# PJLab-ADG/neuralsim

Measured on NVIDIA H100. Metric: Mrays/sec fwd+bwd, higher is better.
Workload: dtype f16

## Files before the change

include/neuralsim_b200.h:

```cpp
#ifndef NEURALSIM_B200_H
#define NEURALSIM_B200_H

#include <stdint.h>

#ifdef __cplusplus
extern "C" {
#endif

#define NSB_MAX_LEVELS 32
#define NSB_MAX_DIMS 4

#define NSB_LOD_DENSE 0
#define NSB_LOD_HASH 7

typedef struct nsb_lotd_meta {
    uint32_t n_dims_to_encode;
    uint32_t n_levels;
    uint32_t n_pseudo_levels;
    uint32_t n_feat_per_pseudo_lvl;
    uint32_t n_encoded_dims;
    uint32_t n_params;
    uint32_t level_res[NSB_MAX_LEVELS][NSB_MAX_DIMS];
    uint32_t level_n_feats[NSB_MAX_LEVELS];
    uint32_t level_types[NSB_MAX_LEVELS];
    uint32_t level_sizes[NSB_MAX_LEVELS];
    uint32_t level_offsets[NSB_MAX_LEVELS + 1];
    uint32_t map_levels[NSB_MAX_LEVELS * 4];
    uint32_t map_cnt[NSB_MAX_LEVELS * 4];
} nsb_lotd_meta;

const char *nsb_last_error(void);
int nsb_version(void);
uint64_t nsb_launch_count(void);
int nsb_set_option(const char *key, int value);

int nsb_lotd_meta_create(int32_t n_dims, int32_t n_levels, const int32_t *lod_res_host,
                         const int32_t *lod_n_feats_host, const int32_t *lod_types_host,
                         uint32_t hashmap_size, nsb_lotd_meta *out_host);

int nsb_lotd_fwd(const nsb_lotd_meta *meta_host, const float *input, const void *params, int params_is_half,
                 int64_t n, int32_t max_level, void *y, float *dy_dx, void *stream);

int nsb_lotd_bwd_grid(const nsb_lotd_meta *meta_host, const void *dL_dy, int dL_dy_is_half, const float *input,
                      int64_t n, int32_t max_level, float scale, float *dL_dparam, void *stream);

int nsb_lotd_bwd_input(const void *dL_dy, int dL_dy_is_half, const float *dy_dx, int64_t n, int32_t n_feat,
                       int32_t n_dims, float scale, float *dL_dx, void *stream);

int nsb_lotd_bwd_bwd_input(const nsb_lotd_meta *meta_host, const float *dL_ddLdx, const void *dL_dy,
                           int dL_dy_is_half, const float *input, const float *dy_dx, int64_t n,
                           int32_t max_level, float scale, float *dL_ddLdy, float *dL_dparam, void *stream);

int nsb_ray_marching(int64_t n_rays, const float *rays_o, const float *rays_d, const float *t_min,
                     const float *t_max, const float *roi, const int32_t *batch_inds, int32_t rx, int32_t ry,
                     int32_t rz, const uint8_t *grid_binary, float step_size, float max_step_size,
                     float dt_gamma, uint32_t max_steps, const int32_t *packed_info, int32_t *num_steps,
                     float *t_starts, float *t_ends, int32_t *ridx, int32_t *gidx, int32_t *bidx, void *stream);
int nsb_ray_marching_listed(int64_t n_rays, const float *rays_o, const float *rays_d, const float *t_min, const float *t_max,
                            const float *roi, const int32_t *batch_inds, int32_t rx, int32_t ry, int32_t rz,
                            const uint8_t *grid_binary, float step_size, float max_step_size, float dt_gamma, uint32_t max_steps,
                            const int32_t *packed_info, int32_t *num_steps, float *t_starts, float *t_ends, int32_t *ridx,
                            int32_t *gidx, int32_t *bidx, const int64_t *ray_list, int64_t n_list, const uint32_t *grid_bits, void *stream);
int nsb_ray_marching_record(int64_t n_rays, const float *rays_o, const float *rays_d, const float *t_min, const float *t_max,
                            const float *roi, int32_t rx, int32_t ry, int32_t rz, const uint8_t *grid_binary, float step_size,
                            float max_step_size, float dt_gamma, uint32_t max_steps, int32_t *num_steps, float *rec_t,
                            const uint32_t *grid_bits, void *stream);
int nsb_march_compact(const float *rec_t, uint32_t max_steps, const int32_t *packed_info, const int64_t *ray_list, int64_t n_list,
                      float *t_starts, int32_t *ridx, void *stream);
int nsb_pack_occ_bits(const uint8_t *grid_binary, int64_t cells, uint32_t *words, void *stream);

enum { NSB_OP_ADD = 0, NSB_OP_SUB, NSB_OP_MUL, NSB_OP_DIV, NSB_OP_GT, NSB_OP_GEQ, NSB_OP_LT, NSB_OP_LEQ,
       NSB_OP_EQ, NSB_OP_NEQ };
int nsb_packed_binary(int op, const float *feats, const float *other, const int64_t *pack_infos, int64_t n_packs,
                      int32_t feat_dim, void *out, void *stream);
int nsb_packed_sum(const float *feats, const int64_t *pack_infos, int64_t n_packs, int32_t feat_dim, float *out,
                   void *stream);
int nsb_packed_cumsum(const float *feats, const int64_t *pack_infos, int64_t n_packs, int32_t feat_dim,
                      int exclusive, int reverse, float *out, void *stream);
int nsb_packed_diff(const float *feats, const int64_t *pack_infos, int64_t n_packs, int32_t feat_dim,
                    const float *appends, const float *last_fill, int backward, float *out, void *stream);
int nsb_packed_searchsorted(const float *bins, const float *vals, const int64_t *pack_infos, int64_t n_packs,
                            int32_t n_vals, int64_t *out_idx, void *stream);
int nsb_packed_invert_cdf(const float *bins, const float *cdfs, const float *u, const int64_t *pack_infos,
                          int64_t n_packs, int32_t n_samples, float *samples, int64_t *bin_idx, void *stream);
int nsb_merge_two_packs_sorted_aligned(const float *vals_a, const int64_t *pack_infos_a, const float *vals_b,
                                       const int64_t *pack_infos_b, const int64_t *pack_infos_out,
                                       int64_t n_packs, int b_sorted, int64_t *pidx_a, int64_t *pidx_b,
                                       void *stream);
int nsb_packed_alpha_to_vw_forward(const float *alphas, const int64_t *pack_infos, int64_t n_packs,
                                   float early_stop_eps, float alpha_thre, float *weights, int64_t *num_steps,
                                   uint8_t *selector, void *stream);
int nsb_packed_alpha_to_vw_backward(const float *weights, const float *grad_weights, const float *alphas,
                                    const int64_t *pack_infos, int64_t n_packs, float early_stop_eps,
                                    float alpha_thre, float *grad_alphas, void *stream);
int nsb_interleave_linstep(const float *start, const int64_t *num_steps, const int64_t *cumsum_steps,
                           const float *step_size, float step_scalar, int64_t n_packs, float *out, int64_t *nidx,
                           void *stream);
int nsb_interleave_arange(const int64_t *num_steps, const int64_t *cumsum_steps, int64_t n_packs, int64_t *out,
                          int64_t *nidx, void *stream);
int nsb_packed_sort(float *vals, const int64_t *pack_infos, int64_t n_packs, int64_t *idx, void *stream);
int nsb_mark_pack_boundaries(const int64_t *ids, int64_t n, int32_t *out, void *stream);

int nsb_sh_encode_forward(const float *inputs, float *outputs, int64_t n, int32_t degree, float *dy_dx,
                          void *stream);
int nsb_sh_encode_backward(const float *grad, const float *dy_dx, int64_t n, int32_t degree, float *grad_inputs,
                           void *stream);

typedef struct nsb_sdf_decoder {
    const void *W1;
    const void *b1;
    const void *W2;
    const void *b2;
    int32_t width;
    float beta;
} nsb_sdf_decoder;

typedef struct nsb_occ_collect {
    float *grid_pcl;
    int32_t res[3];
    float inv_s;
} nsb_occ_collect;

int nsb_fused_sdf(const nsb_lotd_meta *meta_host, const void *params_half, const nsb_sdf_decoder *dec_host,
                  const float *x, int64_t n, int32_t max_level, float *sdf, void *h_out_half, void *stream);
int nsb_fused_sdf_collect(const nsb_lotd_meta *meta_host, const void *params_half, const nsb_sdf_decoder *dec_host, const float *x,
                          const float *rays_o, const float *rays_d, const int64_t *ridx, const float *t, int64_t n,
                          const int64_t *pack_infos, const int64_t *pack_ray, const int64_t *pack_order, int64_t n_packs, int32_t mode,
                          int32_t max_level, float *sdf, const nsb_occ_collect *collect, void *stream);

int nsb_fused_sdf_rays(const nsb_lotd_meta *meta_host, const void *params_half, const nsb_sdf_decoder *dec_host,
                       const float *rays_o, const float *rays_d, const int64_t *ridx, const float *t, int64_t n,
                       int32_t max_level, float *sdf, void *stream);

int nsb_fused_sdf_packs(const nsb_lotd_meta *meta_host, const void *params_half, const nsb_sdf_decoder *dec_host, const float *rays_o,
                        const float *rays_d, const int64_t *pack_infos, const int64_t *pack_ray, int64_t n_packs, const float *t,
                        int32_t max_level, float *sdf, void *stream);

int nsb_fused_sdf_bwd(const nsb_lotd_meta *meta_host, const void *params_half, const nsb_sdf_decoder *dec_host,
                      const float *x, const float *rays_o, const float *rays_d, const int64_t *ridx, const float *t,
                      const float *d_sdf, int64_t n, int32_t max_level, float *d_grid, float *d_W1, float *d_b1,
                      float *d_W2, float *d_b2, void *stream);

int nsb_fused_sdf_bwd_indexed(const nsb_lotd_meta *meta_host, const void *params_half, const nsb_sdf_decoder *dec_host,
                              const float *x, const float *rays_o, const float *rays_d, const int64_t *ridx, const float *t,
                              const float *d_sdf, const int64_t *keep, int64_t n, int32_t max_level, float *d_grid, float *d_W1,
                              float *d_b1, float *d_W2, float *d_b2, void *stream);

int nsb_bind_device_counts(const int64_t *count0, const int64_t *count1);
int nsb_flag_nonzero(const float *v, int64_t n, int32_t *flag, void *stream);
int nsb_query_counts(int64_t *counts, int32_t phase, int32_t n_coarse, const int32_t *n_fine_host, int32_t n_stage, int64_t march_cap,
                     int64_t kept_cap, void *stream);

int nsb_neus_upsample_cdf(const float *sdf, const float *depth, const int64_t *pack_infos, int64_t n_packs, float inv_s,
                          int use_estimate_alpha, float early_stop_eps, float alpha_thre, float *cdf, void *stream);
int nsb_packed_invert_cdf_shared_u(const float *bins, const float *cdfs, const float *u, const int64_t *pack_infos, int64_t n_packs,
                                   int32_t n_samples, float *samples, void *stream);
int nsb_neus_alpha_forward(const float *sdf, const int64_t *pack_infos, int64_t n_packs, const float *inv_s_dev, float early_stop_eps,
                           float alpha_thre, float *alpha, uint8_t *selector, int32_t *num_steps, void *stream);
int nsb_neus_alpha_backward(const float *sdf, const int64_t *pack_infos, int64_t n_packs, const float *inv_s_dev, const float *d_alpha,
                            float *d_sdf, float *d_inv_s, void *stream);
int nsb_composite_forward(const float *alpha, const float *t, const float *rgb, const float *nablas, const int64_t *pack_infos,
                          int64_t n_packs, float early_stop_eps, float alpha_thre, int normalize_depth, const int64_t *ray_index,
                          float *vw, float *mask, float *depth, float *rgb_out, float *nablas_out, void *stream);
int nsb_composite_backward(const float *alpha, const float *t, const float *rgb, const float *nablas, const float *vw,
                           const int64_t *pack_infos, int64_t n_packs, float early_stop_eps, float alpha_thre, int normalize_depth,
                           const float *mask, const float *depth, const float *g_mask, const float *g_depth, const float *g_rgb,
                           const float *g_nablas, const float *g_vw, const int64_t *ray_index, float *d_alpha, float *d_rgb,
                           float *d_nablas, void *stream);

int nsb_scan_counts(const int32_t *counts, int64_t n, int32_t *first, int32_t *info2, int64_t *nz_index, int64_t *nz_pack,
                    const int64_t *src, int64_t *nz_src, int64_t *totals, const int64_t *extra_src, int64_t ticket,
                    void *workspace_zeroed, void *stream);
int64_t nsb_scan_workspace_bytes(void);
int nsb_merge_sorted_vals(const float *dep_a, const float *sdf_a, const int64_t *pack_infos_a, const float *dep_b, const float *sdf_b,
                          int64_t n_packs, int32_t n_b, float *dep_m, float *sdf_m, int64_t *pack_infos_m, void *stream);
int nsb_assemble_boundary(const float *coarse, int64_t n_rays, int32_t n_coarse, const int64_t *ridx_hit, int64_t n_hit, const float *fine,
                          int32_t n_fine, const int32_t *run_len_host, int32_t n_runs, float *d1, float *mid, int64_t *ridx_all,
                          int64_t *pack_infos, void *stream);
int nsb_compact_samples(const uint8_t *selector, const int64_t *pack_infos, const int32_t *first_out, const int32_t *kept, int64_t n_packs,
                        const int64_t *ridx_all, const float *t, const float *alpha, int64_t *pidx, int64_t *ridx_c, float *t_c,
                        float *alpha_c, void *stream);
int nsb_scatter_f32(const float *src, const int64_t *idx, int64_t n, float *dst, void *stream);
int nsb_ray_test_aabb(const float *rays_o, const float *rays_d, int64_t n, const float *center3, const float *radius3, int has_near,
                      float near_clip, int has_far, float far_clip, float *o_n, float *d_n, float *near, float *far, int32_t *flag,
                      int64_t *coherent_pairs, int64_t *row_len, void *stream);
int nsb_ray_block_order(const int64_t *pix, const int64_t *via, int64_t n_packs, int64_t n_rays, const int64_t *pairs, const int64_t *row_len,
                        int64_t *order, void *stream);
int nsb_gather_rays(const int64_t *idx, int64_t n, const float *o_n, const float *d_n, const float *near, const float *far, float *o_c,
                    float *d_c, float *near_c, float *far_c, const float *extra, float *extra_c, int32_t extra_cols, void *stream);

int nsb_occ_ema_update(const float *pts, const float *val, int64_t n, int32_t val_is_sdf, float inv_s, int32_t rx, int32_t ry, int32_t rz,
                       float *pcl_or_null, float *occ_val_grid, uint8_t *occ_grid, uint32_t *occ_bits_or_null, float ema_decay, float occ_thre,
                       float *scratch_cells, void *stream);

typedef struct nsb_color_net {
    const void *W1, *b1, *W2, *b2;
    const void *R1, *rb1, *R2, *rb2, *R3, *rb3;
    int32_t width, rad_width, rad_in, n_appear;
    float beta;
    float nablas_scale[3];
} nsb_color_net;

int64_t nsb_color_tile_bytes(int64_t n);
int nsb_fused_color_fwd(const nsb_lotd_meta *meta_host, const void *params_half, const nsb_color_net *net_host, const float *x,
                        const float *rays_o, const float *rays_d, const int64_t *ridx, const float *t, const float *view_dirs,
                        const float *h_appear, int64_t n, int32_t max_level, float *sdf, float *nablas, float *rgb, float *x_out,
                        void *act_z, void *act_x, void *act_y1, void *act_y2, const nsb_occ_collect *collect, void *stream);
int nsb_fused_color_bwd(const nsb_lotd_meta *meta_host, const void *params_half, const nsb_color_net *net_host, const float *x,
                        const float *rays_o, const float *rays_d, const int64_t *ridx, const float *t, int64_t n, int32_t max_level,
                        const void *act_z, const void *act_x, const void *act_y1, const void *act_y2, const float *rgb,
                        const float *g_sdf, const float *g_nablas, const float *g_rgb, float *dh_scratch, float *d_grid, float *d_W1,
                        float *d_b1, float *d_W2, float *d_b2, float *d_R1, float *d_rb1, float *d_R2, float *d_rb2, float *d_R3,
                        float *d_rb3, void *stream);

int nsb_upsample_rays(const nsb_lotd_meta *meta_host, const void *params_half, const nsb_sdf_decoder *dec_host, const float *rays_o,
                      const float *rays_d, const float *t_starts, const int64_t *pack_infos, const int64_t *ridx_hit, int64_t n_hit,
                      int32_t max_level, int32_t n_stage, const int32_t *n_fine_host, const float *inv_s_stage_host,
                      const float *const *u_stage_host, int32_t use_estimate_alpha, float early_stop_eps, float alpha_thre, float *fine_all,
                      int32_t *overflow, float *scratch, int32_t long_cap, const nsb_occ_collect *collect, void *stream);
int64_t nsb_upsample_rays_scratch_floats(int64_t n_hit_capacity, int32_t long_cap);
int nsb_upsample_persistent(const nsb_lotd_meta *meta_host, const void *params_half, const nsb_sdf_decoder *dec_host, const float *rays_o,
                            const float *rays_d, const float *t_starts, const int64_t *pack_infos, const int64_t *ridx_hit, int64_t n_hit,
                            int32_t max_level, int32_t n_stage, const int32_t *n_fine, const float *inv_s_stage, const float *const *u_stage,
                            int32_t use_estimate_alpha, float early_stop_eps, float alpha_thre, float *fine_all, int32_t *overflow, void *stream);

int nsb_mc_lattice_points(const float *lin0, const float *lin1, const float *lin2, int32_t n1, int32_t n2, int64_t start, int64_t n, float *x,
                          void *stream);
int nsb_mc_count(const float *sdf_win, int32_t w0, int32_t n_win, int32_t n0, int32_t n1, int32_t n2, int32_t p0, int32_t p1, double level,
                 uint8_t *flags, int32_t *vcount, uint8_t *cases, int32_t *tcount, void *stream);
int nsb_mc_vertices(const float *sdf_win, int32_t w0, int32_t n_win, int32_t n0, int32_t n1, int32_t n2, int32_t p0, int32_t p1, double level,
                    const double *bmin3_host, const double *spacing3_host, const uint8_t *flags, const int32_t *vfirst, float *verts, float *normals,
                    void *stream);
int nsb_mc_triangles(int32_t n0, int32_t n1, int32_t n2, int32_t p0, int32_t p1, const uint8_t *cases, const int32_t *tcount, const int32_t *tfirst,
                     const uint8_t *flags, const int32_t *vfirst, int64_t vbase, const uint8_t *carry_flags, const int32_t *carry_first,
                     int64_t carry_base, int32_t *faces, void *stream);

#ifdef __cplusplus
}
#endif
#endif
```

neuralsim_b200/csrc/neus_fused.cu:

```cuda
#include "neus_device.cuh"

namespace nsb {

constexpr int kNB = 256;
__device__ __forceinline__ int64_t gwarp() { return ((int64_t)blockIdx.x * blockDim.x + threadIdx.x) >> 5; }
__device__ __forceinline__ int64_t nwarps() { return ((int64_t)gridDim.x * blockDim.x) >> 5; }
inline unsigned pack_grid(int64_t n_packs) { return wave_grid(n_packs * 32, kNB, 8); }

__global__ void __launch_bounds__(kNB)
k_upsample_cdf(const float *__restrict__ sdf, const float *__restrict__ dep, const int64_t *__restrict__ pi, int64_t n_packs, float inv_s,
               int use_estimate, float eps, float thre, float *__restrict__ cdf, const int64_t *__restrict__ n_dev) {
    const int lane = threadIdx.x & 31;
    n_packs = eff_n(n_packs, n_dev);
    for (int64_t p = gwarp(); p < n_packs; p += nwarps()) {
        const int64_t b = pi[2 * p], n = pi[2 * p + 1];
        float T = 1.f, carry = 0.f, last_excl = 0.f;
        bool stopped = false;
        int cnt = 0;
        for (int64_t k0 = 0; k0 < n; k0 += 32) {
            const int64_t k = k0 + lane;
            float a = 0.f;
            if (k < n) a = use_estimate ? upsample_alpha_at(sdf, dep, b, n, k, inv_s) : neus_alpha_at(sdf, b, n, k, inv_s);
            float w;
            bool sel;
            replay_chunk(a, (int)min((int64_t)32, n - k0), lane, eps, thre, T, stopped, cnt, w, sel);
            const float inc = warp_scan_incl(w, lane) + carry;
            const float excl = inc - w;
            if (k < n) cdf[b + k] = excl;
            if (k == n - 1) last_excl = excl;
            carry = __shfl_sync(0xffffffffu, inc, 31);
        }
        last_excl = __shfl_sync(0xffffffffu, last_excl, (int)((n - 1) & 31));
        const float norm = fmaxf(last_excl, 1e-5f);
        __syncwarp();
        for (int64_t k = lane; k < n; k += 32) cdf[b + k] = __fdiv_rn(cdf[b + k], norm);
    }
}

__global__ void __launch_bounds__(256)
k_invert_cdf_shared_u(const float *__restrict__ bins, const float *__restrict__ cdfs, const float *__restrict__ u, const int64_t *__restrict__ pi,
                      int64_t n_packs, int n_s, float *__restrict__ samples, const int64_t *__restrict__ n_dev) {
    n_packs = eff_n(n_packs, n_dev);
    const int64_t total = n_packs * n_s, stride = (int64_t)gridDim.x * blockDim.x;
    for (int64_t t = (int64_t)blockIdx.x * blockDim.x + threadIdx.x; t < total; t += stride) {
        const int64_t p = t / n_s;
        const int64_t b = pi[2 * p];
        const uint32_t n = (uint32_t)pi[2 * p + 1];
        if (n == 0) { samples[t] = __int_as_float(0x7fc00000); continue; }
        const float *bb = bins + b, *cc = cdfs + b;
        const float uu = u[t - p * n_s];
        uint32_t first = 0, count = n;
        while (count > 0) {
            const uint32_t step = count >> 1, it = first + step;
            if (cc[it] < uu) { first = it + 1; count -= step + 1; } else count = step;
        }
        const uint32_t pos = min(first, n - 1);
        float r;
        if (pos == 0) r = bb[0];
        else {
            const float c0 = cc[pos - 1], pmf = __fsub_rn(cc[pos], c0);
            r = pmf < 1.0e-5f ? bb[pos - 1] : __fmaf_rn(__fdiv_rn(__fsub_rn(uu, c0), pmf), __fsub_rn(bb[pos], bb[pos - 1]), bb[pos - 1]);
        }
        samples[t] = r;
    }
}

__global__ void __launch_bounds__(kNB)
k_neus_alpha_fwd(const float *__restrict__ sdf, const int64_t *__restrict__ pi, int64_t n_packs, const float *__restrict__ inv_s_p, float eps,
                 float thre, float *__restrict__ alpha, uint8_t *__restrict__ selector, int32_t *__restrict__ num_steps,
                 const int64_t *__restrict__ n_dev) {
    const int lane = threadIdx.x & 31;
    const float inv_s = inv_s_p[0];
    if (n_dev) {
        const int64_t live = eff_n(n_packs, n_dev);
        for (int64_t p = live + (int64_t)blockIdx.x * blockDim.x + threadIdx.x; p < n_packs; p += (int64_t)gridDim.x * blockDim.x) num_steps[p] = 0;
        n_packs = live;
    }
    for (int64_t p = gwarp(); p < n_packs; p += nwarps()) {
        const int64_t b = pi[2 * p], n = pi[2 * p + 1];
        float T = 1.f;
        bool stopped = false;
        int cnt = 0;
        for (int64_t k0 = 0; k0 < n; k0 += 32) {
            const int64_t k = k0 + lane;
            const float a = (k < n) ? neus_alpha_at(sdf, b, n, k, inv_s) : 0.f;
            float w;
            bool sel;
            replay_chunk(a, (int)min((int64_t)32, n - k0), lane, eps, thre, T, stopped, cnt, w, sel);
            if (k < n) { alpha[b + k] = a; selector[b + k] = sel ? 1 : 0; }
        }
        if (lane == 0) num_steps[p] = cnt;
    }
}

__global__ void __launch_bounds__(kNB)
k_neus_alpha_bwd(const float *__restrict__ sdf, const int64_t *__restrict__ pi, int64_t n_packs, const float *__restrict__ inv_s_p,
                 const float *__restrict__ d_alpha, float *__restrict__ d_sdf, float *__restrict__ d_inv_s, const int64_t *__restrict__ n_dev) {
    const int lane = threadIdx.x & 31;
    const float inv_s = inv_s_p[0];
    n_packs = eff_n(n_packs, n_dev);
    float acc_invs = 0.f;
    for (int64_t p = gwarp(); p < n_packs; p += nwarps()) {
        const int64_t b = pi[2 * p], n = pi[2 * p + 1];
        for (int64_t k = lane; k < n; k += 32) {
            const float g_own = (k < n - 1) ? d_alpha[b + k] : 0.f, g_prev = (k > 0) ? d_alpha[b + k - 1] : 0.f;
            if (g_own == 0.f && g_prev == 0.f) { d_sdf[b + k] = 0.f; continue; }
            const float s = sdf[b + k];
            const float c = sigmoidf_(s * inv_s);
            float gc = 0.f;
            if (k < n - 1) {
                const float c1 = sigmoidf_(sdf[b + k + 1] * inv_s);
                const float den = c + 1e-5f;
                if ((c - c1) / den >= 0.f) gc += g_own * (c1 + 1e-5f) / (den * den);
            }
            if (k > 0) {
                const float cp = sigmoidf_(sdf[b + k - 1] * inv_s);
                const float den = cp + 1e-5f;
                if ((cp - c) / den >= 0.f) gc -= g_prev / den;
            }
            const float dc = c * (1.f - c);
            d_sdf[b + k] = gc * dc * inv_s;
            acc_invs += gc * dc * s;
        }
    }
    acc_invs = warp_sum(acc_invs);
    if (lane == 0 && acc_invs != 0.f) atomicAdd(d_inv_s, acc_invs);
}

__global__ void __launch_bounds__(kNB)
k_composite_fwd(const float *__restrict__ alpha, const float *__restrict__ t, const float *__restrict__ rgb, const float *__restrict__ nab,
                const int64_t *__restrict__ pi, int64_t n_packs, float eps, float thre, int normalize_depth, const int64_t *__restrict__ ray_index,
                float *__restrict__ vw, float *__restrict__ mask, float *__restrict__ depth, float *__restrict__ rgb_out, float *__restrict__ nab_out,
                const int64_t *__restrict__ n_dev) {
    const int lane = threadIdx.x & 31;
    n_packs = eff_n(n_packs, n_dev);
    for (int64_t p = gwarp(); p < n_packs; p += nwarps()) {
        const int64_t b = pi[2 * p], n = pi[2 * p + 1];
        float T = 1.f;
        bool stopped = false;
        int cnt = 0;
        float sm = 0.f, sd = 0.f, sr[3] = {0.f, 0.f, 0.f}, sn[3] = {0.f, 0.f, 0.f};
        for (int64_t k0 = 0; k0 < n; k0 += 32) {
            const int64_t k = k0 + lane;
            const float a = (k < n) ? alpha[b + k] : 0.f;
            float w;
            bool sel;
            replay_chunk(a, (int)min((int64_t)32, n - k0), lane, eps, thre, T, stopped, cnt, w, sel);
            if (k < n) {
                vw[b + k] = w;
                sm += w;
                sd = fmaf(w, t[b + k], sd);
                if (rgb) { sr[0] = fmaf(w, rgb[(b + k) * 3], sr[0]); sr[1] = fmaf(w, rgb[(b + k) * 3 + 1], sr[1]); sr[2] = fmaf(w, rgb[(b + k) * 3 + 2], sr[2]); }
                if (nab) { sn[0] = fmaf(w, nab[(b + k) * 3], sn[0]); sn[1] = fmaf(w, nab[(b + k) * 3 + 1], sn[1]); sn[2] = fmaf(w, nab[(b + k) * 3 + 2], sn[2]); }
            }
        }
        sm = warp_sum(sm); sd = warp_sum(sd);
#pragma unroll
        for (int c = 0; c < 3; ++c) { sr[c] = warp_sum(sr[c]); sn[c] = warp_sum(sn[c]); }
        if (lane == 0) {
            const int64_t o = ray_index ? ray_index[p] : p;
            mask[o] = sm;
            depth[o] = normalize_depth ? sd / (sm + 1e-10f) : sd;
            if (rgb) { rgb_out[o * 3] = sr[0]; rgb_out[o * 3 + 1] = sr[1]; rgb_out[o * 3 + 2] = sr[2]; }
            if (nab) { nab_out[o * 3] = sn[0]; nab_out[o * 3 + 1] = sn[1]; nab_out[o * 3 + 2] = sn[2]; }
        }
    }
}

__global__ void __launch_bounds__(kNB)
k_composite_bwd(const float *__restrict__ alpha, const float *__restrict__ t, const float *__restrict__ rgb, const float *__restrict__ nab,
                const float *__restrict__ vw, const int64_t *__restrict__ pi, int64_t n_packs, float eps, float thre, int normalize_depth,
                const float *__restrict__ mask, const float *__restrict__ depth, const float *__restrict__ g_mask, const float *__restrict__ g_depth,
                const float *__restrict__ g_rgb, const float *__restrict__ g_nab, const float *__restrict__ g_vw_ext,
                const int64_t *__restrict__ ray_index, float *__restrict__ d_alpha, float *__restrict__ d_rgb, float *__restrict__ d_nab,
                const int64_t *__restrict__ n_dev) {
    const int lane = threadIdx.x & 31;
    n_packs = eff_n(n_packs, n_dev);
    for (int64_t p = gwarp(); p < n_packs; p += nwarps()) {
        const int64_t b = pi[2 * p], n = pi[2 * p + 1];
        const int64_t o = ray_index ? ray_index[p] : p;
        const float gm = g_mask ? g_mask[o] : 0.f, gd = g_depth ? g_depth[o] : 0.f;
        const float M = mask[o], Dp = depth[o];
        const float inv = normalize_depth ? 1.f / (M + 1e-10f) : 1.f;
        float gr[3] = {0.f, 0.f, 0.f}, gn[3] = {0.f, 0.f, 0.f};
        if (g_rgb) { gr[0] = g_rgb[o * 3]; gr[1] = g_rgb[o * 3 + 1]; gr[2] = g_rgb[o * 3 + 2]; }
        if (g_nab) { gn[0] = g_nab[o * 3]; gn[1] = g_nab[o * 3 + 1]; gn[2] = g_nab[o * 3 + 2]; }
        float accum = 0.f;
        for (int64_t k = lane; k < n; k += 32) {
            const float w = vw[b + k];
            float gw = gm + gd * (normalize_depth ? (t[b + k] - Dp) * inv : t[b + k]);
            if (g_vw_ext) gw += g_vw_ext[b + k];
            if (rgb) {
                gw += gr[0] * rgb[(b + k) * 3] + gr[1] * rgb[(b + k) * 3 + 1] + gr[2] * rgb[(b + k) * 3 + 2];
                d_rgb[(b + k) * 3] = w * gr[0]; d_rgb[(b + k) * 3 + 1] = w * gr[1]; d_rgb[(b + k) * 3 + 2] = w * gr[2];
            }
            if (nab) {
                gw += gn[0] * nab[(b + k) * 3] + gn[1] * nab[(b + k) * 3 + 1] + gn[2] * nab[(b + k) * 3 + 2];
                d_nab[(b + k) * 3] = w * gn[0]; d_nab[(b + k) * 3 + 1] = w * gn[1]; d_nab[(b + k) * 3 + 2] = w * gn[2];
            }
            d_alpha[b + k] = gw;
            accum += gw * w;
        }
        accum = warp_sum(accum);
        __syncwarp();
        float T = 1.f;
        bool stopped = false;
        for (int64_t k0 = 0; k0 < n; k0 += 32) {
            const int64_t k = k0 + lane;
            const float a = (k < n) ? alpha[b + k] : 0.f;
            const float gw = (k < n) ? d_alpha[b + k] : 0.f;
            const float gww = (k < n) ? gw * vw[b + k] : 0.f;
            float my_g = 0.f;
            if (!stopped) {
                const int lim = (int)min((int64_t)32, n - k0);
                for (int q = 0; q < lim; ++q) {
                    const float aq = __shfl_sync(0xffffffffu, a, q);
                    const float gq = __shfl_sync(0xffffffffu, gww, q);
                    if (T < eps) { stopped = true; break; }
                    if (aq < thre) continue;
                    if (q == lane) my_g = __fdiv_rn(gw * T - accum, fmaxf(1.f - aq, 1e-10f));
                    accum -= gq;
                    T *= (1.f - aq);
                }
            }
            if (k < n) d_alpha[b + k] = my_g;
        }
    }
}

}

using namespace nsb;
#define STREAM ((cudaStream_t)stream)

extern "C" int nsb_neus_upsample_cdf(const float *sdf, const float *depth, const int64_t *pack_infos, int64_t n_packs, float inv_s,
                                     int use_estimate_alpha, float early_stop_eps, float alpha_thre, float *cdf, void *stream) {
    const DevCounts dn = take_counts();
    if (n_packs == 0) return 0;
    NSB_REQUIRE(sdf && depth && pack_infos && cdf, "nsb_neus_upsample_cdf: NULL argument");
    k_upsample_cdf<<<pack_grid(n_packs), kNB, 0, STREAM>>>(sdf, depth, pack_infos, n_packs, inv_s, use_estimate_alpha, early_stop_eps, alpha_thre, cdf, dn.a);
    return check_launch("nsb_neus_upsample_cdf");
}

extern "C" int nsb_packed_invert_cdf_shared_u(const float *bins, const float *cdfs, const float *u, const int64_t *pack_infos, int64_t n_packs,
                                              int32_t n_samples, float *samples, void *stream) {
    const DevCounts dn = take_counts();
    if (n_packs == 0 || n_samples == 0) return 0;
    NSB_REQUIRE(bins && cdfs && u && pack_infos && samples, "nsb_packed_invert_cdf_shared_u: NULL argument");
    k_invert_cdf_shared_u<<<wave_grid(n_packs * n_samples, 256, 8), 256, 0, STREAM>>>(bins, cdfs, u, pack_infos, n_packs, n_samples, samples, dn.a);
    return check_launch("nsb_packed_invert_cdf_shared_u");
}

extern "C" int nsb_neus_alpha_forward(const float *sdf, const int64_t *pack_infos, int64_t n_packs, const float *inv_s_dev, float early_stop_eps,
                                      float alpha_thre, float *alpha, uint8_t *selector, int32_t *num_steps, void *stream) {
    const DevCounts dn = take_counts();
    if (n_packs == 0) return 0;
    NSB_REQUIRE(sdf && pack_infos && inv_s_dev && alpha && selector && num_steps, "nsb_neus_alpha_forward: NULL argument");
    k_neus_alpha_fwd<<<pack_grid(n_packs), kNB, 0, STREAM>>>(sdf, pack_infos, n_packs, inv_s_dev, early_stop_eps, alpha_thre, alpha, selector, num_steps, dn.a);
    return check_launch("nsb_neus_alpha_forward");
}

extern "C" int nsb_neus_alpha_backward(const float *sdf, const int64_t *pack_infos, int64_t n_packs, const float *inv_s_dev, const float *d_alpha,
                                       float *d_sdf, float *d_inv_s, void *stream) {
    const DevCounts dn = take_counts();
    if (n_packs == 0) return 0;
    NSB_REQUIRE(sdf && pack_infos && inv_s_dev && d_alpha && d_sdf && d_inv_s, "nsb_neus_alpha_backward: NULL argument");
    k_neus_alpha_bwd<<<pack_grid(n_packs), kNB, 0, STREAM>>>(sdf, pack_infos, n_packs, inv_s_dev, d_alpha, d_sdf, d_inv_s, dn.a);
    return check_launch("nsb_neus_alpha_backward");
}

extern "C" int nsb_composite_forward(const float *alpha, const float *t, const float *rgb, const float *nablas, const int64_t *pack_infos,
                                     int64_t n_packs, float early_stop_eps, float alpha_thre, int normalize_depth, const int64_t *ray_index,
                                     float *vw, float *mask, float *depth, float *rgb_out, float *nablas_out, void *stream) {
    const DevCounts dn = take_counts();
    if (n_packs == 0) return 0;
    NSB_REQUIRE(alpha && t && pack_infos && vw && mask && depth, "nsb_composite_forward: NULL argument");
    NSB_REQUIRE((!rgb || rgb_out) && (!nablas || nablas_out), "nsb_composite_forward: missing output buffer");
    k_composite_fwd<<<pack_grid(n_packs), kNB, 0, STREAM>>>(alpha, t, rgb, nablas, pack_infos, n_packs, early_stop_eps, alpha_thre, normalize_depth,
                                                            ray_index, vw, mask, depth, rgb_out, nablas_out, dn.a);
    return check_launch("nsb_composite_forward");
}

extern "C" int nsb_composite_backward(const float *alpha, const float *t, const float *rgb, const float *nablas, const float *vw,
                                      const int64_t *pack_infos, int64_t n_packs, float early_stop_eps, float alpha_thre, int normalize_depth,
                                      const float *mask, const float *depth, const float *g_mask, const float *g_depth, const float *g_rgb,
                                      const float *g_nablas, const float *g_vw, const int64_t *ray_index, float *d_alpha, float *d_rgb,
                                      float *d_nablas, void *stream) {
    const DevCounts dn = take_counts();
    if (n_packs == 0) return 0;
    NSB_REQUIRE(alpha && t && vw && pack_infos && mask && depth && d_alpha, "nsb_composite_backward: NULL argument");
    NSB_REQUIRE((!rgb || d_rgb) && (!nablas || d_nablas), "nsb_composite_backward: missing output buffer");
    k_composite_bwd<<<pack_grid(n_packs), kNB, 0, STREAM>>>(alpha, t, rgb, nablas, vw, pack_infos, n_packs, early_stop_eps, alpha_thre, normalize_depth,
                                                            mask, depth, g_mask, g_depth, g_rgb, g_nablas, g_vw, ray_index, d_alpha, d_rgb, d_nablas, dn.a);
    return check_launch("nsb_composite_backward");
}
```

neuralsim_b200/csrc/neus_glue.cu:

```cuda
#include "nsb_common.cuh"

namespace nsb {

__device__ __forceinline__ int64_t gwarp_() { return ((int64_t)blockIdx.x * blockDim.x + threadIdx.x) >> 5; }
__device__ __forceinline__ int64_t nwarps_() { return ((int64_t)gridDim.x * blockDim.x) >> 5; }

constexpr int kScanT = 1024, kScanI = 8, kScanMaxBlocks = 128;
struct ScanWs {
    long long sum[kScanMaxBlocks];
    int nz[kScanMaxBlocks];
    int flag[kScanMaxBlocks];
    int ticket;
};

__device__ __forceinline__ void block_scan_pair(int64_t &ps, int32_t &pz, int lane, int warp, int64_t *s_sum, int32_t *s_nz) {
#pragma unroll
    for (int o = 1; o < 32; o <<= 1) {
        const int64_t a = __shfl_up_sync(0xffffffffu, ps, o);
        const int32_t b = __shfl_up_sync(0xffffffffu, pz, o);
        if (lane >= o) { ps += a; pz += b; }
    }
    __syncthreads();
    if (lane == 31) { s_sum[warp] = ps; s_nz[warp] = pz; }
    __syncthreads();
    if (warp == 0) {
        int64_t a = s_sum[lane];
        int32_t b = s_nz[lane];
#pragma unroll
        for (int o = 1; o < 32; o <<= 1) {
            const int64_t a2 = __shfl_up_sync(0xffffffffu, a, o);
            const int32_t b2 = __shfl_up_sync(0xffffffffu, b, o);
            if (lane >= o) { a += a2; b += b2; }
        }
        s_sum[lane] = a;
        s_nz[lane] = b;
    }
    __syncthreads();
}

__global__ void __launch_bounds__(kScanT)
k_scan_counts(const int32_t *__restrict__ counts, int64_t n, int64_t seg, ScanWs *__restrict__ ws, int32_t *__restrict__ first,
              int32_t *__restrict__ info2, int64_t *__restrict__ nz_index, int64_t *__restrict__ nz_pack, const int64_t *__restrict__ src,
              int64_t *__restrict__ nz_src, int64_t *totals, const int64_t *__restrict__ extra_src, int64_t ticket) {
    __shared__ int64_t s_sum[32];
    __shared__ int32_t s_nz[32];
    __shared__ int64_t s_carry_sum;
    __shared__ int32_t s_carry_nz;
    __shared__ int s_b;
    if (threadIdx.x == 0) s_b = atomicAdd(&ws->ticket, 1);
    __syncthreads();
    const int tid = threadIdx.x, lane = tid & 31, warp = tid >> 5, b = s_b;
    const int64_t lo = (int64_t)b * seg, hi = min(n, lo + seg);
    int64_t ps = 0;
    int32_t pz = 0;
    for (int64_t i = lo + tid; i < hi; i += kScanT) { const int32_t c = counts[i]; ps += c; pz += c > 0 ? 1 : 0; }
    block_scan_pair(ps, pz, lane, warp, s_sum, s_nz);
    const int64_t my_sum = s_sum[31];
    const int32_t my_nz = s_nz[31];
    if (tid == 0) {
        ws->sum[b] = my_sum;
        ws->nz[b] = my_nz;
        __threadfence();
        atomicExch(&ws->flag[b], 1);
    }
    ps = 0;
    pz = 0;
    if (tid < b) {
        while (atomicAdd(&ws->flag[tid], 0) == 0) {}
        __threadfence();
        ps = *((volatile long long *)&ws->sum[tid]);
        pz = *((volatile int *)&ws->nz[tid]);
    }
    block_scan_pair(ps, pz, lane, warp, s_sum, s_nz);
    if (tid == 0) { s_carry_sum = s_sum[31]; s_carry_nz = s_nz[31]; }
    __syncthreads();
    int64_t carry_sum = s_carry_sum;
    int32_t carry_nz = s_carry_nz;
    if (b == gridDim.x - 1 && tid == 0) {
        volatile int64_t *tv = totals;
        tv[0] = carry_sum + my_sum;
        tv[1] = carry_nz + my_nz;
        if (extra_src) tv[2] = extra_src[0];
        if (ticket) {
            __threadfence_system();
            tv[3] = ticket;
        }
    }
    for (int64_t base = lo; base < hi; base += (int64_t)kScanT * kScanI) {
        const int64_t i0 = base + (int64_t)tid * kScanI;
        int32_t c[kScanI];
        ps = 0;
        pz = 0;
#pragma unroll
        for (int k = 0; k < kScanI; ++k) {
            c[k] = (i0 + k < hi) ? counts[i0 + k] : 0;
            ps += c[k];
            pz += c[k] > 0 ? 1 : 0;
        }
        const int64_t tsum = ps;
        const int32_t tnz = pz;
        block_scan_pair(ps, pz, lane, warp, s_sum, s_nz);
        int64_t excl = carry_sum + (warp ? s_sum[warp - 1] : 0) + ps - tsum;
        int32_t rank = carry_nz + (warp ? s_nz[warp - 1] : 0) + pz - tnz;
#pragma unroll
        for (int k = 0; k < kScanI; ++k) {
            const int64_t i = i0 + k;
            if (i < hi) {
                if (first) first[i] = (int32_t)excl;
                if (info2) { info2[2 * i] = (int32_t)excl; info2[2 * i + 1] = c[k]; }
                if (c[k] > 0) {
                    if (nz_index) nz_index[rank] = i;
                    if (nz_pack) { nz_pack[2 * rank] = excl; nz_pack[2 * rank + 1] = c[k]; }
                    if (nz_src) nz_src[rank] = src[i];
                    ++rank;
                }
            }
            excl += c[k];
        }
        carry_sum += s_sum[31];
        carry_nz += s_nz[31];
    }
}

constexpr int kMergeWarps = 8;
__global__ void __launch_bounds__(kMergeWarps * 32)
k_merge_vals(const float *__restrict__ dep_a, const float *__restrict__ sdf_a, const int64_t *__restrict__ pi_a, const float *__restrict__ dep_b,
             const float *__restrict__ sdf_b, int64_t n_packs, int nb, float *__restrict__ dep_m, float *__restrict__ sdf_m,
             int64_t *__restrict__ pi_m, const int64_t *__restrict__ n_dev) {
    extern __shared__ float s_b[];
    n_packs = eff_n(n_packs, n_dev);
    const int lane = threadIdx.x & 31, w = threadIdx.x >> 5;
    float *bb = s_b + w * nb;
    for (int64_t p = gwarp_(); p < n_packs; p += nwarps_()) {
        const int64_t a0 = pi_a[2 * p], na = pi_a[2 * p + 1];
        const int64_t m0 = a0 + p * nb;
        __syncwarp();
        for (int j = lane; j < nb; j += 32) bb[j] = dep_b[p * nb + j];
        __syncwarp();
        if (lane == 0) { pi_m[2 * p] = m0; pi_m[2 * p + 1] = na + nb; }
        for (int64_t i = lane; i < na; i += 32) {
            const float v = dep_a[a0 + i];
            int lo = 0, cnt = nb;
            while (cnt > 0) {
                const int step = cnt >> 1;
                if (bb[lo + step] <= v) { lo += step + 1; cnt -= step + 1; } else cnt = step;
            }
            dep_m[m0 + i + lo] = v;
            if (sdf_m) sdf_m[m0 + i + lo] = sdf_a[a0 + i];
        }
        for (int j = lane; j < nb; j += 32) {
            const float v = bb[j];
            int64_t lo = 0, cnt = na;
            while (cnt > 0) {
                const int64_t step = cnt >> 1;
                if (dep_a[a0 + lo + step] < v) { lo += step + 1; cnt -= step + 1; } else cnt = step;
            }
            dep_m[m0 + j + lo] = v;
            if (sdf_m) sdf_m[m0 + j + lo] = sdf_b[p * nb + j];
        }
    }
}

constexpr int kAsmWarps = 8, kAsmMaxRuns = 8, kAsmChunk = 8;
struct AsmRuns { int n, len[kAsmMaxRuns]; };

__device__ __forceinline__ int count_less(const float *a, int n, float v, bool or_equal) {
    int lo = 0, cnt = n;
    while (cnt > 0) {
        const int step = cnt >> 1;
        const float u = a[lo + step];
        if (or_equal ? (u <= v) : (u < v)) { lo += step + 1; cnt -= step + 1; } else cnt = step;
    }
    return lo;
}

__global__ void __launch_bounds__(kAsmWarps * 32)
k_assemble_boundary(const float *__restrict__ coarse, int64_t n_rays, int nc, const int64_t *__restrict__ ridx_hit, int64_t n_hit,
                    const float *__restrict__ fine, int nf, const AsmRuns runs, float *__restrict__ d1, float *__restrict__ mid,
                    int64_t *__restrict__ ridx_all, int64_t *__restrict__ pack_infos, const int64_t *__restrict__ n_rays_dev,
                    const int64_t *__restrict__ n_hit_dev) {
    extern __shared__ float s_v[];
    static_assert(kAsmChunk >= 1 && kAsmChunk <= 32, "one candidate per lane");
    n_rays = eff_n(n_rays, n_rays_dev);
    n_hit = eff_n(n_hit, n_hit_dev);
    const int lane = threadIdx.x & 31, w = threadIdx.x >> 5, cap = nc + nf;
    float *raw = s_v + (size_t)w * 2 * cap, *srt = raw + cap;
    const int64_t n_chunks = (n_rays + kAsmChunk - 1) / kAsmChunk;
    for (int64_t c = gwarp_(); c < n_chunks; c += nwarps_()) {
        const int64_t r0 = c * kAsmChunk;
        int64_t lo0 = 0, cnt = n_hit;
        while (cnt > 0) {
            const int64_t step = cnt >> 1;
            if (ridx_hit[lo0 + step] < r0) { lo0 += step + 1; cnt -= step + 1; } else cnt = step;
        }
        long long cand = -1;
        if (lane < kAsmChunk && lo0 + lane < n_hit) cand = ridx_hit[lo0 + lane];
        int used = 0;
        for (int j = 0; j < kAsmChunk; ++j) {
            const int64_t r = r0 + j;
            if (r >= n_rays) break;
            const bool hit = __shfl_sync(0xffffffffu, cand, used) == r;
            const int64_t lo = lo0 + used;
            const int n = nc + (hit ? nf : 0);
            const int64_t first = (int64_t)nc * r + (int64_t)nf * lo;
            if (lane == 0) { pack_infos[2 * r] = first; pack_infos[2 * r + 1] = n; }
            if (!hit) {
                for (int k = lane; k < nc; k += 32) {
                    const float v = coarse[r * nc + k];
                    const float diff = (k < nc - 1) ? __fsub_rn(coarse[r * nc + k + 1], v) : 0.f;
                    d1[first + k] = v;
                    mid[first + k] = __fadd_rn(v, __fmul_rn(diff, 0.5f));
                    ridx_all[first + k] = r;
                }
                continue;
            }
            ++used;
            __syncwarp();
            for (int k = lane; k < nc; k += 32) raw[k] = coarse[r * nc + k];
            for (int k = lane; k < nf; k += 32) raw[nc + k] = fine[lo * nf + k];
            __syncwarp();
            for (int e = lane; e < n; e += 32) {
                const float v = raw[e];
                int rank = 0, start = 0;
                for (int q = -1; q < runs.n; ++q) {
                    const int len = q < 0 ? nc : runs.len[q];
                    if (e >= start && e < start + len) rank += e - start;
                    else rank += count_less(raw + start, len, v, start < e);
                    start += len;
                }
                srt[rank] = v;
            }
            __syncwarp();
            for (int k = lane; k < n; k += 32) {
                const float v = srt[k];
                const float diff = (k < n - 1) ? __fsub_rn(srt[k + 1], v) : 0.f;
                d1[first + k] = v;
                mid[first + k] = __fadd_rn(v, __fmul_rn(diff, 0.5f));
                ridx_all[first + k] = r;
            }
        }
    }
}

__global__ void __launch_bounds__(256)
k_compact_samples(const uint8_t *__restrict__ selector, const int64_t *__restrict__ pi, const int32_t *__restrict__ first_out,
                  const int32_t *__restrict__ kept, int64_t n_packs, const int64_t *__restrict__ ridx_all, const float *__restrict__ t,
                  const float *__restrict__ alpha, int64_t *__restrict__ pidx, int64_t *__restrict__ ridx_c, float *__restrict__ t_c,
                  float *__restrict__ alpha_c, const int64_t *__restrict__ n_dev) {
    const int lane = threadIdx.x & 31;
    n_packs = eff_n(n_packs, n_dev);
    for (int64_t p = gwarp_(); p < n_packs; p += nwarps_()) {
        const int32_t kp = kept[p];
        if (kp == 0) continue;
        const int64_t b = pi[2 * p], n = pi[2 * p + 1];
        int64_t out = first_out[p];
        int32_t done = 0;
        for (int64_t k0 = 0; k0 < n && done < kp; k0 += 32) {
            const int64_t k = k0 + lane;
            const bool sel = k < n && selector[b + k] != 0;
            const uint32_t m = __ballot_sync(0xffffffffu, sel);
            if (sel) {
                const int64_t o = out + __popc(m & ((1u << lane) - 1u));
                pidx[o] = b + k;
                ridx_c[o] = ridx_all[b + k];
                t_c[o] = t[b + k];
                alpha_c[o] = alpha[b + k];
            }
            const int c = __popc(m);
            out += c;
            done += c;
        }
    }
}

__global__ void __launch_bounds__(256)
k_scatter_f32(const float *__restrict__ src, const int64_t *__restrict__ idx, int64_t n, float *__restrict__ dst, const int64_t *__restrict__ n_dev) {
    n = eff_n(n, n_dev);
    const int64_t stride = (int64_t)gridDim.x * blockDim.x;
    for (int64_t j = (int64_t)blockIdx.x * blockDim.x + threadIdx.x; j < n; j += stride) dst[idx[j]] = src[j];
}


__device__ __forceinline__ float min_nan(float a, float b) { return (a != a || b != b) ? __int_as_float(0x7fc00000) : fminf(a, b); }
__device__ __forceinline__ float max_nan(float a, float b) { return (a != a || b != b) ? __int_as_float(0x7fc00000) : fmaxf(a, b); }

struct RayTestArgs {
    float c[3], r[3];
    float near_clip, far_clip;
    int has_near, has_far;
};

__global__ void __launch_bounds__(256)
k_ray_test_aabb(const float *__restrict__ rays_o, const float *__restrict__ rays_d, int64_t n, const RayTestArgs a, float *__restrict__ o_n,
                float *__restrict__ d_n, float *__restrict__ near, float *__restrict__ far, int32_t *__restrict__ flag,
                unsigned long long *__restrict__ coherent_pairs, unsigned long long *__restrict__ row_len) {
    const int64_t stride = (int64_t)gridDim.x * blockDim.x;
    unsigned int close = 0;
    for (int64_t i = (int64_t)blockIdx.x * blockDim.x + threadIdx.x; i < n; i += stride) {
        if (row_len && i >= 2) {
            float rev = 0.f;
#pragma unroll
            for (int d = 0; d < 3; ++d) rev += (rays_d[i * 3 + d] - rays_d[(i - 1) * 3 + d]) * (rays_d[3 + d] - rays_d[d]);
            if (rev < 0.f) atomicMin(row_len, (unsigned long long)i);
        }
        if (coherent_pairs && i > 0) {
            float dd = 0.f, od = 0.f;
#pragma unroll
            for (int d = 0; d < 3; ++d) {
                dd = fmaxf(dd, fabsf(rays_d[i * 3 + d] - rays_d[(i - 1) * 3 + d]));
                od = fmaxf(od, fabsf(rays_o[i * 3 + d] - rays_o[(i - 1) * 3 + d]) / a.r[d]);
            }
            const float len = fmaxf(fmaxf(fabsf(rays_d[i * 3]), fabsf(rays_d[i * 3 + 1])), fabsf(rays_d[i * 3 + 2]));
            close += (dd <= 0.03f * len && od <= 0.03f) ? 1u : 0u;
        }
        float tn = 0.f, tf = 0.f;
#pragma unroll
        for (int d = 0; d < 3; ++d) {
            const float o = __fdiv_rn(__fsub_rn(rays_o[i * 3 + d], a.c[d]), a.r[d]);
            const float v = __fdiv_rn(rays_d[i * 3 + d], a.r[d]);
            o_n[i * 3 + d] = o;
            d_n[i * 3 + d] = v;
            const float ta = __fdiv_rn(__fsub_rn(-1.f, o), v), tb = __fdiv_rn(__fsub_rn(1.f, o), v);
            const float lo = min_nan(ta, tb), hi = max_nan(ta, tb);
            tn = d == 0 ? lo : max_nan(tn, lo);
            tf = d == 0 ? hi : min_nan(tf, hi);
        }
        if (a.has_near && tn == tn) tn = fmaxf(tn, a.near_clip);
        if (a.has_far && tf == tf) tf = fminf(tf, a.far_clip);
        bool m = (tf > tn) && (tf > (a.has_near ? a.near_clip : 0.f));
        if (a.has_far) m = m && (tn < a.far_clip);
        near[i] = tn;
        far[i] = tf;
        flag[i] = m ? 1 : 0;
    }
    if (coherent_pairs) {
        close = __reduce_add_sync(0xffffffffu, close);
        if ((threadIdx.x & 31) == 0 && close) atomicAdd(coherent_pairs, (unsigned long long)close);
    }
}

constexpr int kOrdT = 256, kOrdMaxBx = 4096;
constexpr int kBlkW = 8, kBlkH = 4;

__device__ __forceinline__ int64_t pixel_of(const int64_t *__restrict__ pix, const int64_t *__restrict__ via, int64_t p) {
    return pix[via ? via[p] : p];
}

__device__ int64_t lower_bound_pixel(const int64_t *__restrict__ pix, const int64_t *__restrict__ via, int64_t n, int64_t key) {
    int64_t lo = 0, hi = n;
    while (lo < hi) {
        const int64_t mid = (lo + hi) >> 1;
        if (pixel_of(pix, via, mid) < key) lo = mid + 1; else hi = mid;
    }
    return lo;
}

__global__ void __launch_bounds__(kOrdT)
k_ray_block_order(const int64_t *__restrict__ pix, const int64_t *__restrict__ via, int64_t n, int64_t n_rays, const int64_t *__restrict__ pairs,
                  const int64_t *__restrict__ row_len, int64_t *__restrict__ order, const int64_t *__restrict__ n_dev) {
    __shared__ uint32_t mask[kOrdMaxBx];
    __shared__ int32_t offs[kOrdMaxBx];
    __shared__ int32_t wsum[kOrdT / 32];
    n = eff_n(n, n_dev);
    const int64_t W = *row_len;
    const bool coherent = n_rays > 64 && 4 * *pairs >= 3 * (n_rays - 1);
    const int64_t nbx = (W + kBlkW - 1) / kBlkW;
    const int tid = threadIdx.x, lane = tid & 31, warp = tid >> 5;
    if (n == 0) return;
    if (!coherent || W < 2 || nbx > kOrdMaxBx) {
        for (int64_t j = (int64_t)blockIdx.x * kOrdT + tid; j < n; j += (int64_t)gridDim.x * kOrdT) order[j] = j;
        return;
    }
    const int64_t rows = kBlkH * W, n_brows = pixel_of(pix, via, n - 1) / rows + 1;
    constexpr int kPer = kOrdMaxBx / kOrdT;
    for (int64_t by = blockIdx.x; by < n_brows; by += gridDim.x) {
        const int64_t lo = lower_bound_pixel(pix, via, n, by * rows), hi = lower_bound_pixel(pix, via, n, (by + 1) * rows);
        for (int64_t b = tid; b < nbx; b += kOrdT) mask[b] = 0u;
        __syncthreads();
        for (int64_t p = lo + tid; p < hi; p += kOrdT) {
            const int64_t q = pixel_of(pix, via, p) - by * rows, py = q / W, px = q - py * W;
            atomicOr(&mask[px / kBlkW], 1u << (py * kBlkW + px % kBlkW));
        }
        __syncthreads();
        int loc = 0;
#pragma unroll
        for (int k = 0; k < kPer; ++k) {
            const int b = tid * kPer + k;
            if (b < nbx) loc += __popc(mask[b]);
        }
        int incl = loc;
#pragma unroll
        for (int o = 1; o < 32; o <<= 1) {
            const int v = __shfl_up_sync(0xffffffffu, incl, o);
            if (lane >= o) incl += v;
        }
        if (lane == 31) wsum[warp] = incl;
        __syncthreads();
        int run = incl - loc;
        for (int w = 0; w < warp; ++w) run += wsum[w];
#pragma unroll
        for (int k = 0; k < kPer; ++k) {
            const int b = tid * kPer + k;
            if (b < nbx) { offs[b] = run; run += __popc(mask[b]); }
        }
        __syncthreads();
        for (int64_t p = lo + tid; p < hi; p += kOrdT) {
            const int64_t q = pixel_of(pix, via, p) - by * rows, py = q / W, px = q - py * W;
            const uint32_t bit = (uint32_t)(py * kBlkW + px % kBlkW);
            order[lo + offs[px / kBlkW] + __popc(mask[px / kBlkW] & ((1u << bit) - 1u))] = p;
        }
        __syncthreads();
    }
}

__global__ void __launch_bounds__(256)
k_gather_rays(const int64_t *__restrict__ idx, int64_t n, const float *__restrict__ o_n, const float *__restrict__ d_n, const float *__restrict__ near,
              const float *__restrict__ far, float *__restrict__ o_c, float *__restrict__ d_c, float *__restrict__ near_c, float *__restrict__ far_c,
              const float *__restrict__ extra, float *__restrict__ extra_c, int extra_cols, const int64_t *__restrict__ n_dev) {
    n = eff_n(n, n_dev);
    const int64_t stride = (int64_t)gridDim.x * blockDim.x;
    for (int64_t j = (int64_t)blockIdx.x * blockDim.x + threadIdx.x; j < n; j += stride) {
        const int64_t i = idx[j];
#pragma unroll
        for (int d = 0; d < 3; ++d) { o_c[j * 3 + d] = o_n[i * 3 + d]; d_c[j * 3 + d] = d_n[i * 3 + d]; }
        near_c[j] = near[i];
        far_c[j] = far[i];
        for (int c = 0; c < extra_cols; ++c) extra_c[j * extra_cols + c] = extra[i * extra_cols + c];
    }
}

__global__ void __launch_bounds__(256)
k_flag_nonzero(const float *__restrict__ v, int64_t n, int32_t *__restrict__ flag, const int64_t *__restrict__ n_dev) {
    const int64_t ne = eff_n(n, n_dev), stride = (int64_t)gridDim.x * blockDim.x;
    for (int64_t i = (int64_t)blockIdx.x * blockDim.x + threadIdx.x; i < n; i += stride) flag[i] = (i < ne && v[i] != 0.f) ? 1 : 0;
}

__global__ void k_query_counts(int64_t *__restrict__ c, int phase, int nc, int n_stage, int nf0, int nf1, int nf2, int nf3, int64_t march_cap,
                               int64_t kept_cap) {
    if (threadIdx.x != 0 || blockIdx.x != 0) return;
    if (phase == 0) {
        const int nf[4] = {nf0, nf1, nf2, nf3};
        int64_t M = c[3], nh = c[4];
        int64_t worst = M, tot = 0;
        for (int q = 0; q + 1 < n_stage; ++q) worst += nh * nf[q];
        if (worst > march_cap) { c[20] |= 1; M = 0; nh = 0; }
        c[12] = M;
        c[13] = nh;
        int64_t merged = M;
        for (int q = 0; q < 4; ++q) {
            c[14 + q] = q < n_stage ? nh * nf[q] : 0;
            if (q < n_stage) tot += nf[q];
            if (q + 1 < n_stage) merged += nh * nf[q];
            c[22 + q] = merged;
        }
        c[18] = c[0] * nc + nh * tot;
    } else {
        int64_t K = c[6], pu = c[7];
        const bool fits = K <= kept_cap;
        if (!fits) { c[20] |= 2; K = 0; pu = 0; }
        c[19] = K;
        c[21] = pu;
        c[26] = fits ? c[0] : 0;
    }
}

}

using namespace nsb;
#define STREAM ((cudaStream_t)stream)

extern "C" int nsb_flag_nonzero(const float *v, int64_t n, int32_t *flag, void *stream) {
    const DevCounts dn = take_counts();
    if (n == 0) return 0;
    NSB_REQUIRE(v && flag, "nsb_flag_nonzero: NULL argument");
    k_flag_nonzero<<<wave_grid(n, 256, 8), 256, 0, STREAM>>>(v, n, flag, dn.a);
    return check_launch("nsb_flag_nonzero");
}

extern "C" int nsb_query_counts(int64_t *counts, int32_t phase, int32_t n_coarse, const int32_t *n_fine_host, int32_t n_stage, int64_t march_cap,
                                int64_t kept_cap, void *stream) {
    NSB_REQUIRE(counts, "nsb_query_counts: counts is NULL");
    NSB_REQUIRE(n_stage >= 0 && n_stage <= 4 && (n_stage == 0 || n_fine_host), "nsb_query_counts: at most 4 up-sampling stages");
    int nf[4] = {0, 0, 0, 0};
    for (int q = 0; q < n_stage; ++q) nf[q] = n_fine_host[q];
    k_query_counts<<<1, 32, 0, STREAM>>>(counts, phase, n_coarse, n_stage, nf[0], nf[1], nf[2], nf[3], march_cap, kept_cap);
    return check_launch("nsb_query_counts");
}

extern "C" int64_t nsb_scan_workspace_bytes(void) { return (int64_t)sizeof(ScanWs); }

extern "C" int nsb_scan_counts(const int32_t *counts, int64_t n, int32_t *first, int32_t *info2, int64_t *nz_index, int64_t *nz_pack,
                               const int64_t *src, int64_t *nz_src, int64_t *totals, const int64_t *extra_src, int64_t ticket,
                               void *workspace_zeroed, void *stream) {
    NSB_REQUIRE(totals && workspace_zeroed, "nsb_scan_counts: totals / workspace is NULL");
    NSB_REQUIRE(n == 0 || counts, "nsb_scan_counts: counts is NULL");
    NSB_REQUIRE(!nz_src || src, "nsb_scan_counts: nz_src needs src");
    int64_t nb = (n + (int64_t)kScanT * kScanI - 1) / ((int64_t)kScanT * kScanI);
    const int64_t cap = sm_count() < kScanMaxBlocks ? sm_count() : kScanMaxBlocks;
    if (nb > cap) nb = cap;
    if (nb < 1) nb = 1;
    int64_t seg = (n + nb - 1) / nb;
    seg = (seg + kScanI - 1) / kScanI * kScanI;
    k_scan_counts<<<(unsigned)nb, kScanT, 0, STREAM>>>(counts, n, seg, (ScanWs *)workspace_zeroed, first, info2, nz_index, nz_pack, src, nz_src, totals, extra_src, ticket);
    return check_launch("nsb_scan_counts");
}

extern "C" int nsb_merge_sorted_vals(const float *dep_a, const float *sdf_a, const int64_t *pack_infos_a, const float *dep_b, const float *sdf_b,
                                     int64_t n_packs, int32_t n_b, float *dep_m, float *sdf_m, int64_t *pack_infos_m, void *stream) {
    const DevCounts dn = take_counts();
    if (n_packs == 0) return 0;
    NSB_REQUIRE(dep_a && pack_infos_a && dep_b && dep_m && pack_infos_m, "nsb_merge_sorted_vals: NULL argument");
    NSB_REQUIRE((sdf_m == nullptr) || (sdf_a && sdf_b), "nsb_merge_sorted_vals: sdf_m needs sdf_a and sdf_b");
    NSB_REQUIRE(n_b > 0 && n_b <= 1024, "nsb_merge_sorted_vals: n_b must be in [1, 1024]");
    const size_t smem = (size_t)kMergeWarps * n_b * sizeof(float);
    k_merge_vals<<<wave_grid(n_packs * 32, kMergeWarps * 32, 8), kMergeWarps * 32, smem, STREAM>>>(dep_a, sdf_a, pack_infos_a, dep_b, sdf_b, n_packs, n_b,
                                                                                                 dep_m, sdf_m, pack_infos_m, dn.a);
    return check_launch("nsb_merge_sorted_vals");
}

extern "C" int nsb_assemble_boundary(const float *coarse, int64_t n_rays, int32_t n_coarse, const int64_t *ridx_hit, int64_t n_hit, const float *fine,
                                     int32_t n_fine, const int32_t *run_len, int32_t n_runs, float *d1, float *mid, int64_t *ridx_all,
                                     int64_t *pack_infos, void *stream) {
    const DevCounts dn = take_counts();
    if (n_rays == 0) return 0;
    NSB_REQUIRE(coarse && d1 && mid && ridx_all && pack_infos, "nsb_assemble_boundary: NULL argument");
    NSB_REQUIRE(n_hit == 0 || (ridx_hit && fine), "nsb_assemble_boundary: hit rays need ridx_hit and fine");
    NSB_REQUIRE(n_coarse > 0 && n_fine >= 0 && n_coarse + n_fine <= 1024, "nsb_assemble_boundary: n_coarse + n_fine must be <= 1024");
    const size_t smem = (size_t)kAsmWarps * 2 * (n_coarse + n_fine) * sizeof(float);
    NSB_REQUIRE(smem <= 96 * 1024, "nsb_assemble_boundary: too many samples per ray for shared memory");
    AsmRuns runs{};
    NSB_REQUIRE(n_runs >= 0 && n_runs <= kAsmMaxRuns && (n_runs == 0 || run_len), "nsb_assemble_boundary: at most %d sorted runs", kAsmMaxRuns);
    int tot = 0;
    for (int q = 0; q < n_runs; ++q) { runs.len[q] = run_len[q]; tot += run_len[q]; }
    runs.n = n_runs;
    NSB_REQUIRE(tot == n_fine, "nsb_assemble_boundary: run lengths must add up to n_fine");
    const unsigned grid = wave_grid(n_rays * 32, kAsmWarps * 32, 8);
    opt_in_smem(k_assemble_boundary, 96 * 1024);
    k_assemble_boundary<<<grid, kAsmWarps * 32, smem, STREAM>>>(coarse, n_rays, n_coarse, ridx_hit, n_hit, fine, n_fine, runs, d1, mid, ridx_all, pack_infos,
                                                               dn.a, dn.b);
    return check_launch("nsb_assemble_boundary");
}

extern "C" int nsb_compact_samples(const uint8_t *selector, const int64_t *pack_infos, const int32_t *first_out, const int32_t *kept, int64_t n_packs,
                                   const int64_t *ridx_all, const float *t, const float *alpha, int64_t *pidx, int64_t *ridx_c, float *t_c,
                                   float *alpha_c, void *stream) {
    const DevCounts dn = take_counts();
    if (n_packs == 0) return 0;
    NSB_REQUIRE(selector && pack_infos && first_out && kept && ridx_all && t && alpha && pidx && ridx_c && t_c && alpha_c,
                "nsb_compact_samples: NULL argument");
    k_compact_samples<<<wave_grid(n_packs * 32, 256, 8), 256, 0, STREAM>>>(selector, pack_infos, first_out, kept, n_packs, ridx_all, t, alpha, pidx, ridx_c,
                                                                          t_c, alpha_c, dn.a);
    return check_launch("nsb_compact_samples");
}

extern "C" int nsb_scatter_f32(const float *src, const int64_t *idx, int64_t n, float *dst, void *stream) {
    const DevCounts dn = take_counts();
    if (n == 0) return 0;
    NSB_REQUIRE(src && idx && dst, "nsb_scatter_f32: NULL argument");
    k_scatter_f32<<<wave_grid(n, 256, 8), 256, 0, STREAM>>>(src, idx, n, dst, dn.a);
    return check_launch("nsb_scatter_f32");
}

extern "C" int nsb_ray_test_aabb(const float *rays_o, const float *rays_d, int64_t n, const float *center3, const float *radius3, int has_near,
                                 float near_clip, int has_far, float far_clip, float *o_n, float *d_n, float *near, float *far, int32_t *flag,
                                 int64_t *coherent_pairs, int64_t *row_len, void *stream) {
    if (n == 0) return 0;
    NSB_REQUIRE(rays_o && rays_d && center3 && radius3 && o_n && d_n && near && far && flag, "nsb_ray_test_aabb: NULL argument");
    RayTestArgs a{{center3[0], center3[1], center3[2]}, {radius3[0], radius3[1], radius3[2]}, near_clip, far_clip, has_near, has_far};
    if (row_len && cudaMemsetAsync(row_len, 0xff, sizeof(int64_t), STREAM) != cudaSuccess) return check_launch("nsb_ray_test_aabb (row length)");
    k_ray_test_aabb<<<wave_grid(n, 256, 8), 256, 0, STREAM>>>(rays_o, rays_d, n, a, o_n, d_n, near, far, flag, (unsigned long long *)coherent_pairs,
                                                           (unsigned long long *)row_len);
    return check_launch("nsb_ray_test_aabb");
}

extern "C" int nsb_ray_block_order(const int64_t *pix, const int64_t *via, int64_t n_packs, int64_t n_rays, const int64_t *pairs, const int64_t *row_len,
                                   int64_t *order, void *stream) {
    const DevCounts dn = take_counts();
    if (n_packs == 0) return 0;
    NSB_REQUIRE(pix && pairs && row_len && order, "nsb_ray_block_order: NULL argument");
    k_ray_block_order<<<wave_grid(n_packs, 4 * 32 * 8, 1), kOrdT, 0, STREAM>>>(pix, via, n_packs, n_rays, pairs, row_len, order, dn.a);
    return check_launch("nsb_ray_block_order");
}

extern "C" int nsb_gather_rays(const int64_t *idx, int64_t n, const float *o_n, const float *d_n, const float *near, const float *far, float *o_c,
                               float *d_c, float *near_c, float *far_c, const float *extra, float *extra_c, int32_t extra_cols, void *stream) {
    const DevCounts dn = take_counts();
    if (n == 0) return 0;
    NSB_REQUIRE(idx && o_n && d_n && near && far && o_c && d_c && near_c && far_c, "nsb_gather_rays: NULL argument");
    NSB_REQUIRE(extra_cols == 0 || (extra && extra_c), "nsb_gather_rays: extra payload needs both pointers");
    k_gather_rays<<<wave_grid(n, 256, 8), 256, 0, STREAM>>>(idx, n, o_n, d_n, near, far, o_c, d_c, near_c, far_c, extra, extra_c, extra_cols, dn.a);
    return check_launch("nsb_gather_rays");
}
```

neuralsim_b200/graphics/neus_fused.py:

```python
from __future__ import annotations

import ctypes

import torch

from .. import _lib as L

__all__ = ["upsample_cdf", "sample_cdf_uniform", "neus_alpha_compress", "neus_alpha_compact", "composite", "scan_counts", "merge_sorted_vals",
           "assemble_boundary", "march_lean", "upsample_rays", "block_order"]

_U_CACHE = {}


def _f32c(t):
    return t.detach().contiguous().float()


@torch.no_grad()
def upsample_cdf(sdf, depth, pack_infos, inv_s: float, use_estimate_alpha=False, early_stop_eps=1e-4, alpha_thre=0.0):
    sdf, depth = _f32c(sdf), _f32c(depth)
    cdf = torch.empty_like(sdf)
    L.check(L.lib().nsb_neus_upsample_cdf(L.ptr(sdf, "f32"), L.ptr(depth, "f32"), L.ptr(pack_infos, "i64"), L.c_i64(pack_infos.shape[0]),
                                          L.c_f32(inv_s), ctypes.c_int(1 if use_estimate_alpha else 0), L.c_f32(early_stop_eps),
                                          L.c_f32(alpha_thre), L.ptr(cdf), L.stream_ptr()), "neus_upsample_cdf")
    return cdf


@torch.no_grad()
def sample_cdf_uniform(bins, cdfs, pack_infos, num_to_sample: int):
    key = (num_to_sample, bins.device)
    u = _U_CACHE.get(key)
    if u is None:
        u = _U_CACHE[key] = torch.linspace(0., 1., num_to_sample + 2, device=bins.device, dtype=torch.float32)[1:-1].contiguous()
    P = pack_infos.shape[0]
    out = torch.empty(P, num_to_sample, device=bins.device, dtype=torch.float32)
    L.check(L.lib().nsb_packed_invert_cdf_shared_u(L.ptr(bins, "f32"), L.ptr(cdfs, "f32"), L.ptr(u, "f32"), L.ptr(pack_infos, "i64"),
                                                   L.c_i64(P), L.c_i32(num_to_sample), L.ptr(out), L.stream_ptr()),
            "packed_invert_cdf_shared_u")
    return out


class _NeusAlpha(torch.autograd.Function):
    @staticmethod
    def forward(ctx, sdf, inv_s, pack_infos, early_stop_eps, alpha_thre):
        sdf_c, inv_c = _f32c(sdf), _f32c(inv_s).reshape(1)
        P = pack_infos.shape[0]
        alpha = torch.empty_like(sdf_c)
        sel = torch.empty(sdf_c.shape[0], dtype=torch.bool, device=sdf_c.device)
        steps = torch.empty(P, dtype=torch.int32, device=sdf_c.device)
        L.check(L.lib().nsb_neus_alpha_forward(L.ptr(sdf_c, "f32"), L.ptr(pack_infos, "i64"), L.c_i64(P), L.ptr(inv_c, "f32"),
                                               L.c_f32(early_stop_eps), L.c_f32(alpha_thre), L.ptr(alpha), L.ptr(sel), L.ptr(steps),
                                               L.stream_ptr()), "neus_alpha_forward")
        ctx.save_for_backward(sdf_c, inv_c, pack_infos)
        ctx.inv_shape = inv_s.shape
        ctx.mark_non_differentiable(sel, steps)
        return alpha, sel, steps

    @staticmethod
    def backward(ctx, g_alpha, _gs, _gn):
        sdf_c, inv_c, pack_infos = ctx.saved_tensors
        g = g_alpha.contiguous().float()
        d_sdf = torch.empty_like(sdf_c)
        d_inv = torch.zeros(1, device=sdf_c.device, dtype=torch.float32)
        L.check(L.lib().nsb_neus_alpha_backward(L.ptr(sdf_c, "f32"), L.ptr(pack_infos, "i64"), L.c_i64(pack_infos.shape[0]),
                                                L.ptr(inv_c, "f32"), L.ptr(g, "f32"), L.ptr(d_sdf), L.ptr(d_inv), L.stream_ptr()),
                "neus_alpha_backward")
        return (d_sdf if ctx.needs_input_grad[0] else None, d_inv.reshape(ctx.inv_shape) if ctx.needs_input_grad[1] else None,
                None, None, None)


def neus_alpha_compress(sdf, inv_s, pack_infos, early_stop_eps=1e-4, alpha_thre=0.0):
    if not isinstance(inv_s, torch.Tensor):
        inv_s = torch.tensor(float(inv_s), device=sdf.device)
    alpha, sel, steps = _NeusAlpha.apply(sdf, inv_s, pack_infos, early_stop_eps, alpha_thre)
    pidx = sel.nonzero()[..., 0]
    nidx = (steps > 0).nonzero()[..., 0]
    kept = steps[nidx].long()
    cs = kept.cumsum(0)
    return alpha, nidx, torch.stack([cs - kept, kept], 1), pidx


class _GatherUnique(torch.autograd.Function):

    @staticmethod
    def forward(ctx, src, pidx, gathered):
        ctx.save_for_backward(pidx)
        ctx.n = src.shape[0]
        return gathered

    @staticmethod
    def backward(ctx, g):
        pidx, = ctx.saved_tensors
        g = g.contiguous().float()
        d = torch.zeros(ctx.n, dtype=torch.float32, device=g.device)
        L.check(L.lib().nsb_scatter_f32(L.ptr(g, "f32"), L.ptr(pidx, "i64"), L.c_i64(pidx.shape[0]), L.ptr(d), L.stream_ptr()), "scatter_f32")
        return d, None, None


_SCAN_WS = []
_HOST_SLOTS = {}


def _host_slot():
    dev = torch.cuda.current_device()
    st = _HOST_SLOTS.get(dev)
    if st is None:
        t = torch.zeros(4, dtype=torch.int64).pin_memory()
        st = _HOST_SLOTS[dev] = [t, t.numpy(), 0]
    return st


def _scan_ws_bytes():
    if not _SCAN_WS:
        L.lib().nsb_scan_workspace_bytes.restype = ctypes.c_int64
        _SCAN_WS.append(int(L.lib().nsb_scan_workspace_bytes()))
    return _SCAN_WS[0]


@torch.no_grad()
def scan_counts(counts, *, want_first=False, want_info2=False, want_index=False, want_pack=False, src=None, extra=None):
    n, dev = counts.shape[0], counts.device
    first = torch.empty(n, dtype=torch.int32, device=dev) if want_first else None
    info2 = torch.empty(n, 2, dtype=torch.int32, device=dev) if want_info2 else None
    index = torch.empty(n, dtype=torch.int64, device=dev) if want_index else None
    pack = torch.empty(n, 2, dtype=torch.int64, device=dev) if want_pack else None
    nz_src = torch.empty(n, dtype=torch.int64, device=dev) if src is not None else None
    slot = _host_slot()
    slot[2] += 1
    ticket = slot[2]
    ws = torch.zeros(_scan_ws_bytes(), dtype=torch.uint8, device=dev)
    L.check(L.lib().nsb_scan_counts(L.ptr(counts, "i32"), L.c_i64(n), L.ptr(first, allow_none=True), L.ptr(info2, allow_none=True),
                                    L.ptr(index, allow_none=True), L.ptr(pack, allow_none=True), L.ptr(src, "i64", allow_none=True),
                                    L.ptr(nz_src, allow_none=True), ctypes.c_void_p(slot[0].data_ptr()), L.ptr(extra, "i64", allow_none=True),
                                    L.c_i64(ticket), L.ptr(ws), L.stream_ptr()), "scan_counts")
    host = slot[1]
    spins = 0
    while host[3] != ticket:
        spins += 1
        if spins > 2_000_000 and spins % 1_000_000 == 0:
            torch.cuda.current_stream().synchronize()
            if host[3] != ticket:
                raise RuntimeError("scan_counts: the kernel finished without publishing its totals")
    total, nnz = int(host[0]), int(host[1])
    out = dict(total=total, n_nonzero=nnz, first=first, info2=info2, extra=[int(host[2])])
    out["index"] = index[:nnz] if index is not None else None
    out["pack"] = pack[:nnz] if pack is not None else None
    out["src"] = nz_src[:nnz] if nz_src is not None else None
    return out


@torch.no_grad()
def block_order(pix, via, rays_row):
    n = pix.shape[0] if via is None else via.shape[0]
    order = torch.empty(n, dtype=torch.int64, device=pix.device)
    n_rays, pr = rays_row
    L.check(L.lib().nsb_ray_block_order(L.ptr(pix, "i64"), L.ptr(via, "i64", allow_none=True), L.c_i64(n), L.c_i64(n_rays), L.ptr(pr, "i64"),
                                        L.ptr(pr[1:], "i64"), L.ptr(order), L.stream_ptr()), "ray_block_order")
    return order


@torch.no_grad()
def merge_sorted_vals(dep_a, sdf_a, pack_infos_a, dep_b, sdf_b):
    P, nb = dep_b.shape
    n = dep_a.shape[0] + P * nb
    dep_m = torch.empty(n, dtype=torch.float32, device=dep_a.device)
    sdf_m = torch.empty_like(dep_m) if sdf_a is not None else None
    pim = torch.empty_like(pack_infos_a)
    L.check(L.lib().nsb_merge_sorted_vals(L.ptr(dep_a, "f32"), L.ptr(sdf_a, "f32", allow_none=True), L.ptr(pack_infos_a, "i64"), L.ptr(dep_b, "f32"),
                                          L.ptr(sdf_b, "f32", allow_none=True), L.c_i64(P), L.c_i32(nb), L.ptr(dep_m), L.ptr(sdf_m, allow_none=True),
                                          L.ptr(pim), L.stream_ptr()), "merge_sorted_vals")
    return dep_m, sdf_m, pim


@torch.no_grad()
def assemble_boundary(coarse, ridx_hit, fine, run_len=None):
    R, nc = coarse.shape
    n_hit, nf = (fine.shape if fine is not None else (0, 0))
    S, dev = R * nc + n_hit * nf, coarse.device
    d1, mid = torch.empty(S, dtype=torch.float32, device=dev), torch.empty(S, dtype=torch.float32, device=dev)
    ridx_all = torch.empty(S, dtype=torch.int64, device=dev)
    pi = torch.empty(R, 2, dtype=torch.int64, device=dev)
    run_len = [nf] if run_len is None else list(run_len)
    rl = (ctypes.c_int32 * len(run_len))(*run_len)
    L.check(L.lib().nsb_assemble_boundary(L.ptr(coarse, "f32"), L.c_i64(R), L.c_i32(nc), L.ptr(ridx_hit, "i64", allow_none=True), L.c_i64(n_hit),
                                          L.ptr(fine, "f32", allow_none=True), L.c_i32(nf), rl, L.c_i32(len(run_len)), L.ptr(d1), L.ptr(mid),
                                          L.ptr(ridx_all), L.ptr(pi), L.stream_ptr()), "assemble_boundary")
    return d1, mid, ridx_all, pi


def neus_alpha_compact(sdf, inv_s, pack_infos, ridx_all, t_mid, rays_inds, early_stop_eps=1e-4, alpha_thre=0.0):
    if not isinstance(inv_s, torch.Tensor):
        inv_s = torch.tensor(float(inv_s), device=sdf.device)
    alpha, sel, steps = _NeusAlpha.apply(sdf, inv_s, pack_infos, early_stop_eps, alpha_thre)
    with torch.no_grad():
        sc = scan_counts(steps, want_first=True, want_index=True, want_pack=True, src=rays_inds)
        K = sc["total"]
        if K == 0:
            return None
        dev = sdf.device
        pidx, ridx_c = torch.empty(K, dtype=torch.int64, device=dev), torch.empty(K, dtype=torch.int64, device=dev)
        t_c, alpha_c = torch.empty(K, dtype=torch.float32, device=dev), torch.empty(K, dtype=torch.float32, device=dev)
        L.check(L.lib().nsb_compact_samples(L.ptr(sel.view(torch.uint8), "u8"), L.ptr(pack_infos, "i64"), L.ptr(sc["first"], "i32"), L.ptr(steps, "i32"),
                                            L.c_i64(pack_infos.shape[0]), L.ptr(ridx_all, "i64"), L.ptr(t_mid, "f32"), L.ptr(alpha.detach(), "f32"),
                                            L.ptr(pidx), L.ptr(ridx_c), L.ptr(t_c), L.ptr(alpha_c), L.stream_ptr()), "compact_samples")
    alpha_k = _GatherUnique.apply(alpha, pidx, alpha_c) if alpha.requires_grad else alpha_c
    return dict(alpha=alpha_k, ridx=ridx_c, t=t_c, pack_infos=sc["pack"], nidx=sc["index"], rays_inds_hit=sc["src"], pidx=pidx)


_BITS_CACHE = {}


@torch.no_grad()
def _occ_bits(occ_grid):
    key = (occ_grid.data_ptr(), occ_grid._version, tuple(occ_grid.shape))
    hit = _BITS_CACHE.get("k")
    if hit is None or hit[0] != key:
        cells = occ_grid.numel()
        words = torch.empty((cells + 31) // 32, dtype=torch.int32, device=occ_grid.device)
        L.check(L.lib().nsb_pack_occ_bits(L.ptr(occ_grid.contiguous().view(torch.uint8), "u8"), L.c_i64(cells), L.ptr(words), L.stream_ptr()), "pack_occ_bits")
        hit = _BITS_CACHE["k"] = (key, words, occ_grid)
    return hit[1]


@torch.no_grad()
def march_lean(occ_grid, rays_o, rays_d, near, far, *, step_size, max_steps, max_step_size=1e10, dt_gamma=0.0, roi=None):
    R, dev = rays_o.shape[0], rays_o.device
    if roi is None:
        roi = torch.tensor([-1, -1, -1, 1, 1, 1], dtype=torch.float32, device=dev)
    g = occ_grid.contiguous().view(torch.uint8)
    res = occ_grid.shape[-3:]
    args = (L.c_i64(R), L.ptr(rays_o, "f32", "rays_o"), L.ptr(rays_d, "f32", "rays_d"), L.ptr(near, "f32", "near"), L.ptr(far, "f32", "far"),
            L.ptr(roi, "f32", "roi"), None, L.c_i32(res[0]), L.c_i32(res[1]), L.c_i32(res[2]), L.ptr(g, "u8"), L.c_f32(step_size),
            L.c_f32(max_step_size), L.c_f32(dt_gamma), ctypes.c_uint32(int(max_steps)))
    num_steps = torch.empty(R, dtype=torch.int32, device=dev)
    bits = _occ_bits(occ_grid) if occ_grid.numel() * 4 // 32 <= 96 * 1024 else None
    with L.KERNEL_TIMER.time("march", R):
        L.check(L.lib().nsb_ray_marching_listed(*args, None, L.ptr(num_steps), None, None, None, None, None, None, L.c_i64(0),
                                                L.ptr(bits, allow_none=True), L.stream_ptr()), "ray_marching")
    sc = scan_counts(num_steps, want_info2=True, want_index=True, want_pack=True)
    M = sc["total"]
    if M == 0:
        return None
    t_starts = torch.empty(M, dtype=torch.float32, device=dev)
    ridx = torch.empty(M, dtype=torch.int32, device=dev)
    with L.KERNEL_TIMER.time("march", R):
        L.check(L.lib().nsb_ray_marching_listed(*args, L.ptr(sc["info2"]), None, L.ptr(t_starts), None, L.ptr(ridx), None, None,
                                                L.ptr(sc["index"], "i64"), L.c_i64(sc["n_nonzero"]), L.ptr(bits, allow_none=True), L.stream_ptr()),
                    "ray_marching")
    return sc["index"], sc["pack"], t_starts, ridx.long()


class _Composite(torch.autograd.Function):
    @staticmethod
    def forward(ctx, alpha, t, rgb, nablas, pack_infos, normalize_depth, early_stop_eps, alpha_thre, ray_index, n_rays):
        a, tt = _f32c(alpha), _f32c(t)
        r = None if rgb is None else _f32c(rgb)
        nb = None if nablas is None else _f32c(nablas)
        P, dev = pack_infos.shape[0], a.device
        vw = torch.empty_like(a)
        n_out = P if ray_index is None else int(n_rays)
        cols = 2 + (3 if r is not None else 0) + (3 if nb is not None else 0)
        buf = (torch.empty if ray_index is None else torch.zeros)(cols * n_out, device=dev)
        mask, depth = buf[:n_out], buf[n_out:2 * n_out]
        rgb_o = buf[2 * n_out:5 * n_out].view(n_out, 3) if r is not None else None
        o3 = 5 * n_out if r is not None else 2 * n_out
        nab_o = buf[o3:o3 + 3 * n_out].view(n_out, 3) if nb is not None else None
        L.check(L.lib().nsb_composite_forward(L.ptr(a, "f32"), L.ptr(tt, "f32"), L.ptr(r, "f32", allow_none=True),
                                              L.ptr(nb, "f32", allow_none=True), L.ptr(pack_infos, "i64"), L.c_i64(P), L.c_f32(early_stop_eps),
                                              L.c_f32(alpha_thre), ctypes.c_int(1 if normalize_depth else 0), L.ptr(ray_index, "i64", allow_none=True),
                                              L.ptr(vw), L.ptr(mask), L.ptr(depth), L.ptr(rgb_o, allow_none=True), L.ptr(nab_o, allow_none=True),
                                              L.stream_ptr()), "composite_forward")
        ctx.save_for_backward(a, tt, r, nb, vw, pack_infos, mask, depth, ray_index)
        ctx.cfg = (normalize_depth, early_stop_eps, alpha_thre)
        ctx.set_materialize_grads(False)
        empty = a.new_empty(0)
        return vw, mask, depth, (rgb_o if rgb_o is not None else empty), (nab_o if nab_o is not None else empty)

    @staticmethod
    def backward(ctx, g_vw, g_mask, g_depth, g_rgb, g_nab):
        a, tt, r, nb, vw, pack_infos, mask, depth, ray_index = ctx.saved_tensors
        normalize_depth, eps, thre = ctx.cfg
        P = pack_infos.shape[0]

        def opt(g, present=True):
            return None if (g is None or not present) else g.contiguous().float()
        g_vw, g_mask, g_depth = opt(g_vw), opt(g_mask), opt(g_depth)
        g_rgb, g_nab = opt(g_rgb, r is not None), opt(g_nab, nb is not None)
        d_alpha = torch.empty_like(a)
        d_rgb = torch.empty_like(r) if r is not None else None
        d_nab = torch.empty_like(nb) if nb is not None else None
        P_ = L.ptr
        L.check(L.lib().nsb_composite_backward(
            P_(a, "f32"), P_(tt, "f32"), P_(r, allow_none=True), P_(nb, allow_none=True), P_(vw, "f32"), P_(pack_infos, "i64"), L.c_i64(P),
            L.c_f32(eps), L.c_f32(thre), ctypes.c_int(1 if normalize_depth else 0), P_(mask), P_(depth), P_(g_mask, allow_none=True),
            P_(g_depth, allow_none=True), P_(g_rgb, allow_none=True), P_(g_nab, allow_none=True), P_(g_vw, allow_none=True),
            P_(ray_index, "i64", allow_none=True), P_(d_alpha), P_(d_rgb, allow_none=True), P_(d_nab, allow_none=True), L.stream_ptr()), "composite_backward")
        return d_alpha, None, d_rgb, d_nab, None, None, None, None, None, None


def composite(alpha, t, pack_infos, rgb=None, nablas=None, normalize_depth=True, early_stop_eps=1e-4, alpha_thre=0.0, ray_index=None,
              n_rays=None):
    vw, mask, depth, rgb_o, nab_o = _Composite.apply(alpha, t, rgb, nablas, pack_infos, normalize_depth, early_stop_eps, alpha_thre,
                                                     ray_index, n_rays)
    return vw, mask, depth, (rgb_o if rgb is not None else None), (nab_o if nablas is not None else None)


def _quantiles(n, dev):
    key = (n, dev)
    u = _U_CACHE.get(key)
    if u is None:
        u = _U_CACHE[key] = torch.linspace(0., 1., n + 2, device=dev, dtype=torch.float32)[1:-1].contiguous()
    return u


@torch.no_grad()
def upsample_rays(meta, grid16, dec, ridx_hit, pack_infos, t_starts, rays_o, rays_d, inv_s_stages, num_fine, *, max_level, max_steps, use_estimate_alpha=False,
                  early_stop_eps=1e-4, alpha_thre=0.0, collect=None, count=None):
    n_hit, dev = ridx_hit.shape[0], t_starts.device
    n_stage = len(num_fine)
    us = [_quantiles(int(n), dev) for n in num_fine]
    fine_all = torch.empty(n_hit, int(sum(num_fine)), dtype=torch.float32, device=dev)
    overflow = torch.zeros(n_hit, dtype=torch.int32, device=dev)
    long_cap = int(max_steps) + int(sum(num_fine[:-1])) + 64
    lib = L.lib()
    lib.nsb_upsample_rays_scratch_floats.restype = ctypes.c_int64
    scratch = torch.empty(int(lib.nsb_upsample_rays_scratch_floats(L.c_i64(n_hit), L.c_i32(long_cap))), dtype=torch.float32, device=dev)
    nf = (ctypes.c_int32 * n_stage)(*[int(n) for n in num_fine])
    invs = (ctypes.c_float * n_stage)(*[float(v) for v in inv_s_stages])
    up = (ctypes.c_void_p * n_stage)(*[u.data_ptr() for u in us])
    if count is not None:
        lib.nsb_bind_device_counts(ctypes.c_void_p(count[0].data_ptr() + 8 * count[1]), ctypes.c_void_p(0))
    try:
        with L.KERNEL_TIMER.time("ray_upsample", n_hit):
            rc = lib.nsb_upsample_rays(meta.c_ref, L.ptr(grid16, "f16"), ctypes.byref(dec), L.ptr(rays_o, "f32"), L.ptr(rays_d, "f32"), L.ptr(t_starts, "f32"),
                                       L.ptr(pack_infos, "i64"), L.ptr(ridx_hit, "i64"), L.c_i64(n_hit), L.c_i32(max_level), L.c_i32(n_stage), nf, invs, up,
                                       L.c_i32(1 if use_estimate_alpha else 0), L.c_f32(early_stop_eps), L.c_f32(alpha_thre), L.ptr(fine_all), L.ptr(overflow),
                                       L.ptr(scratch), L.c_i32(long_cap), ctypes.byref(collect) if collect is not None else None, L.stream_ptr())
    finally:
        if count is not None:
            lib.nsb_bind_device_counts(ctypes.c_void_p(0), ctypes.c_void_p(0))
    L.check(rc, "upsample_rays")
    return fine_all, overflow


@torch.no_grad()
def upsample_persistent(surface, ridx_hit, pack_infos, t_starts, rays_o, rays_d, inv_s_stages, num_fine, use_estimate_alpha=False,
                        early_stop_eps=1e-4, alpha_thre=0.0, max_level=None):
    grid16, dec = surface._fused_state()
    n_hit, dev = ridx_hit.shape[0], t_starts.device
    n_stage = len(num_fine)
    us = []
    for n in num_fine:
        key = (n, dev)
        u = _U_CACHE.get(key)
        if u is None:
            u = _U_CACHE[key] = torch.linspace(0., 1., n + 2, device=dev, dtype=torch.float32)[1:-1].contiguous()
        us.append(u)
    fine_all = torch.empty(n_hit, int(sum(num_fine)), dtype=torch.float32, device=dev)
    overflow = torch.zeros(n_hit, dtype=torch.int32, device=dev)
    nf = (ctypes.c_int32 * n_stage)(*[int(n) for n in num_fine])
    invs = (ctypes.c_float * n_stage)(*[float(v) for v in inv_s_stages])
    up = (ctypes.c_void_p * n_stage)(*[u.data_ptr() for u in us])
    L.check(L.lib().nsb_upsample_persistent(surface.encoding.meta.c_ref, L.ptr(grid16, "f16"), ctypes.byref(dec), L.ptr(rays_o, "f32"), L.ptr(rays_d, "f32"),
                                            L.ptr(t_starts, "f32"), L.ptr(pack_infos, "i64"), L.ptr(ridx_hit, "i64"), L.c_i64(n_hit),
                                            L.c_i32(surface._ml(max_level)), L.c_i32(n_stage), nf, invs, up, L.c_i32(1 if use_estimate_alpha else 0),
                                            L.c_f32(early_stop_eps), L.c_f32(alpha_thre), L.ptr(fine_all), L.ptr(overflow), L.stream_ptr()),
            "upsample_persistent")
    return fine_all, overflow
```

neuralsim_b200/graphics/neus_static.py:

```python
from __future__ import annotations

import ctypes

import torch
import torch.nn.functional as F

from .. import _lib as L
from .raysample import batch_sample_step_linear
from .pack_ops import get_pack_infos_from_batch
from . import neus_fused as NF

__all__ = ["render_static", "StaticFrame", "CNT_SLOTS"]

CNT_SLOTS = dict(n_rays=0, pairs=2, marched_raw=3, hit_raw=4, kept_raw=6, kept_rays_raw=7, nonzero=9, marched=12, hit=13, fine0=14,
                 boundary=18, kept=19, overflow=20, kept_rays=21, merged0=22, rays_if_kept_fits=26, row_len=27)
_NULL = ctypes.c_void_p(0)
MARCH_ONEPASS = "auto"
MARCH_ONEPASS_MAX_BYTES = 64 << 20


def march_onepass(n_rays, max_steps):
    if MARCH_ONEPASS == "0":
        return False
    return MARCH_ONEPASS == "1" or 4 * int(n_rays) * int(max_steps) <= MARCH_ONEPASS_MAX_BYTES


def _slot(cnt, k):
    return ctypes.c_void_p(cnt.data_ptr() + 8 * k)


def _call(fn, what, cnt, k0, k1, *args):
    lib = L.lib()
    lib.nsb_bind_device_counts(_slot(cnt, k0), _slot(cnt, k1) if k1 is not None else _NULL)
    try:
        rc = fn(*args)
    finally:
        lib.nsb_bind_device_counts(_NULL, _NULL)
    L.check(rc, what)


def _scan(counts, cnt, slot, *, first=None, info2=None, index=None, pack=None, src=None, nz_src=None, ws=None):
    if ws is None:
        ws = torch.zeros(NF._scan_ws_bytes(), dtype=torch.uint8, device=counts.device)
    P = L.ptr
    L.check(L.lib().nsb_scan_counts(P(counts, "i32"), L.c_i64(counts.shape[0]), P(first, allow_none=True), P(info2, allow_none=True),
                                    P(index, allow_none=True), P(pack, allow_none=True), P(src, "i64", allow_none=True), P(nz_src, allow_none=True),
                                    _slot(cnt, slot), None, L.c_i64(0), P(ws), L.stream_ptr()), "scan_counts")


def _query_counts(cnt, phase, n_coarse1, num_fine, march_cap, kept_cap):
    nf = (ctypes.c_int32 * max(len(num_fine), 1))(*[int(n) for n in num_fine])
    L.check(L.lib().nsb_query_counts(ctypes.c_void_p(cnt.data_ptr()), L.c_i32(phase), L.c_i32(n_coarse1), nf, L.c_i32(len(num_fine)),
                                     L.c_i64(march_cap), L.c_i64(kept_cap), L.stream_ptr()), "query_counts")


def _sdf_launch(meta, grid16, dec, rays_o, rays_d, t, sdf, *, ridx=None, packs=None, ml, collect, cnt, slot, timer="lotd_gather"):
    P = L.ptr
    mode = 2 if packs is not None else 1
    with L.KERNEL_TIMER.time(timer, t.numel()):
        _call(L.lib().nsb_fused_sdf_collect, "fused_sdf", cnt, slot, None,
              meta.c_ref, P(grid16, "f16"), ctypes.byref(dec), None, P(rays_o, "f32"), P(rays_d, "f32"),
              P(ridx, "i64") if mode == 1 else None, P(t, "f32"), L.c_i64(t.numel()),
              P(packs[0], "i64") if mode == 2 else None, P(packs[1], "i64", allow_none=True) if mode == 2 else None,
              P(packs[2], "i64", allow_none=True) if mode == 2 and len(packs) > 2 else None,
              L.c_i64(packs[0].shape[0] if mode == 2 else 0), L.c_i32(mode), L.c_i32(ml), P(sdf),
              ctypes.byref(collect) if collect is not None else None, L.stream_ptr())
    return sdf


def _block_order(rays_inds, via, n_rays, cnt, slot):
    n = rays_inds.shape[0] if via is None else via.shape[0]
    order = torch.empty(n, dtype=torch.int64, device=rays_inds.device)
    _call(L.lib().nsb_ray_block_order, "ray_block_order", cnt, slot, None, L.ptr(rays_inds, "i64"), L.ptr(via, "i64", allow_none=True), L.c_i64(n),
          L.c_i64(n_rays), _slot(cnt, CNT_SLOTS["pairs"]), _slot(cnt, CNT_SLOTS["row_len"]), L.ptr(order), L.stream_ptr())
    return order


class _StaticSDF(torch.autograd.Function):

    @staticmethod
    def forward(ctx, st, ridx, t, packs, count_slot, grid, W1, b1, W2, b2):
        sdf = torch.empty(t.numel(), dtype=torch.float32, device=t.device)
        _sdf_launch(st.meta, st.grid16, st.dec, st.rays_o, st.rays_d, t, sdf, ridx=ridx if packs is None else None, packs=packs, ml=st.ml,
                    collect=st.collect, cnt=st.cnt, slot=count_slot, timer="fused_sdf_fwd")
        ctx.st, ctx.ridx, ctx.t = st, ridx, t
        ctx.shapes = (grid.shape, W1.shape, b1.shape, W2.shape, b2.shape)
        return sdf

    @staticmethod
    @torch.autograd.function.once_differentiable
    def backward(ctx, d_sdf):
        st, dev = ctx.st, d_sdf.device
        gs, w1s, b1s, w2s, b2s = ctx.shapes
        d_grid = torch.zeros(gs, dtype=torch.float32, device=dev)
        ks = [int(torch.Size(x).numel()) for x in (w1s, b1s, w2s, b2s)]
        small = torch.zeros(sum(ks), dtype=torch.float32, device=dev)
        d_W1, d_b1 = small[:ks[0]].view(w1s), small[ks[0]:ks[0] + ks[1]].view(b1s)
        d_W2, d_b2 = small[ks[0] + ks[1]:ks[0] + ks[1] + ks[2]].view(w2s), small[ks[0] + ks[1] + ks[2]:].view(b2s)
        d_sdf = d_sdf.contiguous().float()
        n = d_sdf.numel()
        P, cnt = L.ptr, st.cnt
        flag = torch.empty(n, dtype=torch.int32, device=dev)
        _call(L.lib().nsb_flag_nonzero, "flag_nonzero", cnt, CNT_SLOTS["boundary"], None, P(d_sdf, "f32"), L.c_i64(n), P(flag), L.stream_ptr())
        keep = torch.empty(n, dtype=torch.int64, device=dev)
        _scan(flag, cnt, CNT_SLOTS["nonzero"], index=keep, ws=st.ws[3])
        with L.KERNEL_TIMER.time("fused_sdf_bwd", n):
            _call(L.lib().nsb_fused_sdf_bwd_indexed, "fused_sdf_bwd", cnt, CNT_SLOTS["nonzero"], None,
                  st.meta.c_ref, P(st.grid16, "f16"), ctypes.byref(st.dec), None, P(st.rays_o, "f32"), P(st.rays_d, "f32"), P(ctx.ridx, "i64"),
                  P(ctx.t, "f32"), P(d_sdf, "f32"), P(keep, "i64"), L.c_i64(n), L.c_i32(st.ml), P(d_grid), P(d_W1), P(d_b1), P(d_W2), P(d_b2),
                  L.stream_ptr())
        return None, None, None, None, None, d_grid, d_W1, d_b1, d_W2, d_b2


class _StaticAlpha(torch.autograd.Function):

    @staticmethod
    def forward(ctx, sdf, inv_s, pack_infos, cnt, early_stop_eps, alpha_thre):
        sdf_c, inv_c = sdf.detach().contiguous().float(), inv_s.detach().contiguous().float().reshape(1)
        Pn, dev = pack_infos.shape[0], sdf_c.device
        alpha = torch.empty_like(sdf_c)
        sel = torch.empty(sdf_c.shape[0], dtype=torch.bool, device=dev)
        steps = torch.empty(Pn, dtype=torch.int32, device=dev)
        P = L.ptr
        _call(L.lib().nsb_neus_alpha_forward, "neus_alpha_forward", cnt, CNT_SLOTS["n_rays"], None, P(sdf_c, "f32"), P(pack_infos, "i64"), L.c_i64(Pn),
              P(inv_c, "f32"), L.c_f32(early_stop_eps), L.c_f32(alpha_thre), P(alpha), P(sel), P(steps), L.stream_ptr())
        ctx.save_for_backward(sdf_c, inv_c, pack_infos)
        ctx.cnt, ctx.inv_shape = cnt, inv_s.shape
        ctx.mark_non_differentiable(sel, steps)
        return alpha, sel, steps

    @staticmethod
    def backward(ctx, g_alpha, _gs, _gn):
        sdf_c, inv_c, pack_infos = ctx.saved_tensors
        g = g_alpha.contiguous().float()
        d_sdf = torch.empty_like(sdf_c)
        d_inv = torch.zeros(1, device=sdf_c.device, dtype=torch.float32)
        P = L.ptr
        _call(L.lib().nsb_neus_alpha_backward, "neus_alpha_backward", ctx.cnt, CNT_SLOTS["n_rays"], None, P(sdf_c, "f32"), P(pack_infos, "i64"),
              L.c_i64(pack_infos.shape[0]), P(inv_c, "f32"), P(g, "f32"), P(d_sdf), P(d_inv), L.stream_ptr())
        return (d_sdf if ctx.needs_input_grad[0] else None, d_inv.reshape(ctx.inv_shape) if ctx.needs_input_grad[1] else None, None, None, None, None)


class _StaticGather(torch.autograd.Function):

    @staticmethod
    def forward(ctx, src, pidx, gathered, cnt):
        ctx.save_for_backward(pidx)
        ctx.n, ctx.cnt = src.shape[0], cnt
        return gathered

    @staticmethod
    def backward(ctx, g):
        pidx, = ctx.saved_tensors
        g = g.contiguous().float()
        d = torch.zeros(ctx.n, dtype=torch.float32, device=g.device)
        P = L.ptr
        _call(L.lib().nsb_scatter_f32, "scatter_f32", ctx.cnt, CNT_SLOTS["kept"], None, P(g, "f32"), P(pidx, "i64"), L.c_i64(pidx.shape[0]), P(d), L.stream_ptr())
        return d, None, None, None


class _StaticColor(torch.autograd.Function):

    @staticmethod
    def forward(ctx, st, ridx, t, view_dirs, h_appear, keep_acts, *params):
        n, dev = t.numel(), t.device
        sdf = torch.empty(n, dtype=torch.float32, device=dev)
        nab = torch.empty(n, 3, dtype=torch.float32, device=dev)
        rgb = torch.empty(n, 3, dtype=torch.float32, device=dev)
        x = torch.empty(n, 3, dtype=torch.float32, device=dev)
        acts = torch.empty(4, int(L.lib().nsb_color_tile_bytes(L.c_i64(n))), dtype=torch.uint8, device=dev) if keep_acts else None
        ap = [L.ptr(acts[k]) if keep_acts else None for k in range(4)]
        P = L.ptr
        with L.KERNEL_TIMER.time("fused_color_fwd", n):
            _call(L.lib().nsb_fused_color_fwd, "fused_color_fwd", st.cnt, CNT_SLOTS["kept"], None,
                  st.meta.c_ref, P(st.grid16, "f16"), ctypes.byref(st.net), None, P(st.rays_o, "f32"), P(st.rays_d, "f32"), P(ridx, "i64"), P(t, "f32"),
                  P(view_dirs, "f32"), P(h_appear, "f32", allow_none=True), L.c_i64(n), L.c_i32(st.ml), P(sdf), P(nab), P(rgb), P(x), *ap,
                  ctypes.byref(st.collect) if st.collect is not None else None, L.stream_ptr())
        ctx.st, ctx.ridx, ctx.t, ctx.n = st, ridx, t, n
        ctx.held = (acts, rgb)
        ctx.shapes = [p.shape for p in params]
        ctx.set_materialize_grads(False)
        ctx.mark_non_differentiable(x)
        return sdf, nab, rgb, x

    @staticmethod
    @torch.autograd.function.once_differentiable
    def backward(ctx, g_sdf, g_nab, g_rgb, _gx):
        acts, rgb = ctx.held
        if acts is None:
            raise RuntimeError("static colour query: backward through a forward that ran without grad")
        st, dev, n = ctx.st, rgb.device, ctx.n
        sizes = [int(torch.Size(s).numel()) for s in ctx.shapes[1:]]
        small = torch.zeros(sum(sizes), dtype=torch.float32, device=dev)
        grads, o = [torch.zeros(ctx.shapes[0], dtype=torch.float32, device=dev)], 0
        for sh, k in zip(ctx.shapes[1:], sizes):
            grads.append(small[o:o + k].view(sh))
            o += k
        if g_sdf is None and g_nab is None and g_rgb is None:
            return (None,) * 6 + tuple(grads)
        c = lambda g: None if g is None else g.contiguous().float()
        g_sdf, g_nab, g_rgb = c(g_sdf), c(g_nab), c(g_rgb)
        dh = torch.empty(n, 32, dtype=torch.float32, device=dev)
        P = L.ptr
        with L.KERNEL_TIMER.time("fused_color_bwd", n):
            _call(L.lib().nsb_fused_color_bwd, "fused_color_bwd", st.cnt, CNT_SLOTS["kept"], None,
                  st.meta.c_ref, P(st.grid16, "f16"), ctypes.byref(st.net), None, P(st.rays_o, "f32"), P(st.rays_d, "f32"), P(ctx.ridx, "i64"),
                  P(ctx.t, "f32"), L.c_i64(n), L.c_i32(st.ml), P(acts[0]), P(acts[1]), P(acts[2]), P(acts[3]), P(rgb), P(g_sdf, allow_none=True),
                  P(g_nab, allow_none=True), P(g_rgb, allow_none=True), P(dh), *[P(g) for g in grads], L.stream_ptr())
        return (None,) * 6 + tuple(grads)


class _StaticComposite(torch.autograd.Function):

    @staticmethod
    def forward(ctx, alpha, t, rgb, nablas, pack_infos, ray_index, n_rays, cnt, normalize_depth, early_stop_eps, alpha_thre):
        a, tt = alpha.detach().contiguous().float(), t.detach().contiguous().float()
        r = None if rgb is None else rgb.detach().contiguous().float()
        nb = None if nablas is None else nablas.detach().contiguous().float()
        Pn, dev = pack_infos.shape[0], a.device
        vw = torch.empty_like(a)
        cols = 2 + (3 if r is not None else 0) + (3 if nb is not None else 0)
        buf = torch.zeros(cols * n_rays, device=dev)
        mask, depth = buf[:n_rays], buf[n_rays:2 * n_rays]
        rgb_o = buf[2 * n_rays:5 * n_rays].view(n_rays, 3) if r is not None else None
        o3 = 5 * n_rays if r is not None else 2 * n_rays
        nab_o = buf[o3:o3 + 3 * n_rays].view(n_rays, 3) if nb is not None else None
        P = L.ptr
        _call(L.lib().nsb_composite_forward, "composite_forward", cnt, CNT_SLOTS["kept_rays"], None, P(a, "f32"), P(tt, "f32"), P(r, "f32", allow_none=True),
              P(nb, "f32", allow_none=True), P(pack_infos, "i64"), L.c_i64(Pn), L.c_f32(early_stop_eps), L.c_f32(alpha_thre),
              ctypes.c_int(1 if normalize_depth else 0), P(ray_index, "i64"), P(vw), P(mask), P(depth), P(rgb_o, allow_none=True),
              P(nab_o, allow_none=True), L.stream_ptr())
        ctx.save_for_backward(a, tt, r, nb, vw, pack_infos, mask, depth, ray_index)
        ctx.cfg = (normalize_depth, early_stop_eps, alpha_thre, cnt)
        ctx.set_materialize_grads(False)
        empty = a.new_empty(0)
        return vw, mask, depth, (rgb_o if rgb_o is not None else empty), (nab_o if nab_o is not None else empty)

    @staticmethod
    def backward(ctx, g_vw, g_mask, g_depth, g_rgb, g_nab):
        a, tt, r, nb, vw, pack_infos, mask, depth, ray_index = ctx.saved_tensors
        normalize_depth, eps, thre, cnt = ctx.cfg

        def opt(g, present=True):
            return None if (g is None or not present) else g.contiguous().float()
        g_vw, g_mask, g_depth = opt(g_vw), opt(g_mask), opt(g_depth)
        g_rgb, g_nab = opt(g_rgb, r is not None), opt(g_nab, nb is not None)
        d_alpha = torch.empty_like(a)
        d_rgb = torch.empty_like(r) if r is not None else None
        d_nab = torch.empty_like(nb) if nb is not None else None
        P = L.ptr
        _call(L.lib().nsb_composite_backward, "composite_backward", cnt, CNT_SLOTS["kept_rays"], None,
              P(a, "f32"), P(tt, "f32"), P(r, allow_none=True), P(nb, allow_none=True), P(vw, "f32"), P(pack_infos, "i64"), L.c_i64(pack_infos.shape[0]),
              L.c_f32(eps), L.c_f32(thre), ctypes.c_int(1 if normalize_depth else 0), P(mask), P(depth), P(g_mask, allow_none=True),
              P(g_depth, allow_none=True), P(g_rgb, allow_none=True), P(g_nab, allow_none=True), P(g_vw, allow_none=True), P(ray_index, "i64"),
              P(d_alpha), P(d_rgb, allow_none=True), P(d_nab, allow_none=True), L.stream_ptr())
        return (d_alpha, None, d_rgb, d_nab) + (None,) * 7


class _State:
    __slots__ = ("meta", "grid16", "dec", "net", "held", "rays_o", "rays_d", "ml", "collect", "cnt", "ws")


def _fp16_images(model):
    s, b = model.implicit_surface, model.radiance_net.blocks.layers
    d = s.decoder.layers
    ps = [s.encoding.flattened_params, d[0].weight, d[0].bias, d[1].weight, d[1].bias, b[0].weight, b[0].bias, b[1].weight, b[1].bias, b[2].weight, b[2].bias]
    t = [torch.empty(p.shape, dtype=torch.half, device=p.device) for p in ps]
    with torch.no_grad():
        t[0].copy_(ps[0].detach())
        torch._foreach_copy_(t[1:], [p.detach() for p in ps[1:]])
    dec = L.SdfDecoderC(t[1].data_ptr(), t[2].data_ptr(), t[3].data_ptr(), t[4].data_ptr(), d[0].out_features, float(d[0].activation.beta))
    r3 = s.radius3d_original
    fk = (r3.data_ptr(), r3._version, float(s.sdf_scale))
    if getattr(model, "_fac_cache", (None,))[0] != fk:
        model._fac_cache = (fk, (s.sdf_scale / r3).float().tolist())
    net = L.ColorNetC(*[x.data_ptr() for x in t[1:]], d[0].out_features, b[0].out_features, b[0].in_features, b[0].in_features - 54,
                      float(d[0].activation.beta), (ctypes.c_float * 3)(*model._fac_cache[1]))
    return t, dec, net, ps


def static_supported(model, cfg):
    qp = dict(model.ray_query_cfg.get("query_param", {}) or {})
    occ = getattr(getattr(model, "accel", None), "occ", None)
    return (getattr(model, "_color_fusable", lambda: False)() and model.use_view_dirs and occ is not None and occ.occ_grid.dim() == 3
            and occ.occ_grid.numel() * 4 // 32 <= 96 * 1024 and qp.get("num_coarse", 0) > 0 and len(qp.get("upsample_inv_s_factors", (1, 4, 16))) <= 4
            and qp.get("coarse_step_cfg", {}).get("step_mode", "linear") == "linear" and (cfg.get("with_rgb", True) or cfg.get("with_normal", True)))


def render_static(model, rays_o, rays_d, rays_h_appear=None, *, near=None, far=None, march_cap, kept_cap, coherent=False, with_rgb=True, with_normal=True,
                  perturb=False, training=None, depth_use_normalized_vw=True, cnt=None):
    P, lib = L.ptr, L.lib()
    if perturb:
        raise RuntimeError("render_static: perturb=True is not built (random streams of capacity-sized draws differ from the reference's); "
                           "use the host-sized path (SingleVolumeRenderer.render)")
    training = model.training if training is None else training
    R, dev = rays_o.shape[0], rays_o.device
    qp = dict(model.ray_query_cfg.get("query_param", {}) or {})
    nc1 = int(qp["num_coarse"]) + 1
    factors = list(qp.get("upsample_inv_s_factors", (1, 4, 16)))
    n_stage = len(factors)
    num_fine = qp.get("num_fine", 8)
    num_fine = [num_fine] * n_stage if isinstance(num_fine, int) else list(num_fine)
    num_fine = [n // 2 * 2 + 1 for n in num_fine]
    nf_tot = int(sum(num_fine))
    upsample_inv_s = qp.get("upsample_inv_s", 64.) / model.upsample_s_divisor
    use_est = bool(qp.get("upsample_use_estimate_alpha", False))
    nablas_has_grad = bool(qp.get("nablas_has_grad", False))
    mc = dict(qp.get("march_cfg", {}))
    fac = mc.pop("step_size_factor", 1.0)
    step_size, dt_gamma = mc.get("step_size", 1e-3) * fac, mc.get("dt_gamma", 0.0) * fac
    max_steps, max_step_size = int(mc.get("max_steps", 512)), mc.get("max_step_size", 1e10)
    march_cap, kept_cap = int(march_cap), int(kept_cap)
    S_cap = R * (nc1 + nf_tot)
    if cnt is None:
        cnt = torch.zeros(32, dtype=torch.int64, device=dev)
    else:
        cnt.zero_()
    st = _State()
    st.cnt = cnt
    wsb = (NF._scan_ws_bytes() + 255) // 256 * 256
    st.ws = torch.zeros(4, wsb, dtype=torch.uint8, device=dev)
    with torch.no_grad():
        t16, st.dec, st.net, masters = _fp16_images(model)
        st.held, st.grid16 = t16, t16[0]
        st.meta = model.implicit_surface.encoding.meta
        st.ml = model.implicit_surface._ml(model.max_level)
        st.collect = model.accel.occ.collect_struct() if training else None
        sp = model.space
        if getattr(sp, "_host_cr", None) is None or sp._host_cr[0] != (sp.aabb.data_ptr(), sp.aabb._version):
            c, r = sp.center.tolist(), sp.radius3d.tolist()
            sp._host_cr = ((sp.aabb.data_ptr(), sp.aabb._version), (ctypes.c_float * 3)(*c), (ctypes.c_float * 3)(*r))
        o_n, d_n = torch.empty(R, 3, device=dev), torch.empty(R, 3, device=dev)
        nr, fr = torch.empty(R, device=dev), torch.empty(R, device=dev)
        flag = torch.empty(R, dtype=torch.int32, device=dev)
        L.check(lib.nsb_ray_test_aabb(P(rays_o.contiguous(), "f32"), P(rays_d.contiguous(), "f32"), L.c_i64(R), sp._host_cr[1], sp._host_cr[2],
                                      ctypes.c_int(0 if near is None else 1), L.c_f32(0. if near is None else near),
                                      ctypes.c_int(0 if far is None else 1), L.c_f32(0. if far is None else far), P(o_n), P(d_n), P(nr), P(fr), P(flag),
                                      _slot(cnt, CNT_SLOTS["pairs"]), _slot(cnt, CNT_SLOTS["row_len"]), L.stream_ptr()), "ray_test_aabb")
        rays_inds = torch.empty(R, dtype=torch.int64, device=dev)
        _scan(flag, cnt, CNT_SLOTS["n_rays"], index=rays_inds, ws=st.ws[0])
        order_b = _block_order(rays_inds, None, R, cnt, CNT_SLOTS["n_rays"]) if coherent else None
        ha = rays_h_appear.detach().contiguous().float() if (rays_h_appear is not None and model.use_h_appear) else None
        if ha is None and model.use_h_appear:
            ha = torch.zeros(R, model.radiance_net.blocks.layers[0].in_features - 54, device=dev)
        n_ha = ha.shape[1] if ha is not None else 0
        rbuf = torch.zeros(R * (8 + n_ha), device=dev)
        o_c, d_c = rbuf[:3 * R].view(R, 3), rbuf[3 * R:6 * R].view(R, 3)
        n_c, f_c = rbuf[6 * R:7 * R], rbuf[7 * R:8 * R]
        ha_c = rbuf[8 * R:].view(R, n_ha) if ha is not None else None
        _call(lib.nsb_gather_rays, "gather_rays", cnt, CNT_SLOTS["n_rays"], None, P(rays_inds, "i64"), L.c_i64(R), P(o_n), P(d_n), P(nr), P(fr), P(o_c), P(d_c),
              P(n_c), P(f_c), P(ha, allow_none=True), P(ha_c, allow_none=True), L.c_i32(0 if ha is None else ha.shape[1]), L.stream_ptr())
        st.rays_o, st.rays_d = o_c, d_c
        view_dirs = (d_c / d_c.norm(dim=-1).clamp_min(1.0e-10).unsqueeze(-1)).contiguous()
        coarse = batch_sample_step_linear(n_c, f_c, nc1, prefix_shape=[R], perturb=perturb).contiguous()
        occ_grid = model.accel.occ.occ_grid
        res = occ_grid.shape[-3:]
        g8 = occ_grid.contiguous().view(torch.uint8)
        bits = torch.empty((occ_grid.numel() + 31) // 32, dtype=torch.int32, device=dev)
        L.check(lib.nsb_pack_occ_bits(P(g8, "u8"), L.c_i64(occ_grid.numel()), P(bits), L.stream_ptr()), "pack_occ_bits")
        roi = torch.tensor([-1, -1, -1, 1, 1, 1], dtype=torch.float32, device=dev) if getattr(model, "_static_roi", None) is None else model._static_roi
        model._static_roi = roi
        margs = (L.c_i64(R), P(o_c, "f32"), P(d_c, "f32"), P(n_c, "f32"), P(f_c, "f32"), P(roi, "f32"), None, L.c_i32(res[0]), L.c_i32(res[1]), L.c_i32(res[2]),
                 P(g8, "u8"), L.c_f32(step_size), L.c_f32(max_step_size), L.c_f32(dt_gamma), ctypes.c_uint32(max_steps))
        num_steps = torch.empty(R, dtype=torch.int32, device=dev)
        rec_t = torch.empty(R * max_steps, dtype=torch.float32, device=dev) if march_onepass(R, max_steps) else None
        with L.KERNEL_TIMER.time("march", R):
            if rec_t is not None:
                _call(lib.nsb_ray_marching_record, "ray_marching_record", cnt, CNT_SLOTS["n_rays"], None, L.c_i64(R), P(o_c, "f32"), P(d_c, "f32"), P(n_c, "f32"),
                      P(f_c, "f32"), P(roi, "f32"), L.c_i32(res[0]), L.c_i32(res[1]), L.c_i32(res[2]), P(g8, "u8"), L.c_f32(step_size), L.c_f32(max_step_size),
                      L.c_f32(dt_gamma), ctypes.c_uint32(max_steps), P(num_steps), P(rec_t), P(bits), L.stream_ptr())
            else:
                _call(lib.nsb_ray_marching_listed, "ray_marching", cnt, CNT_SLOTS["n_rays"], None, *margs, None, P(num_steps), None, None, None, None, None, None,
                      L.c_i64(0), P(bits), L.stream_ptr())
        info2 = torch.empty(R, 2, dtype=torch.int32, device=dev)
        ridx_hit = torch.empty(R, dtype=torch.int64, device=dev)
        pack_infos = torch.empty(R, 2, dtype=torch.int64, device=dev)
        _scan(num_steps, cnt, CNT_SLOTS["marched_raw"], info2=info2, index=ridx_hit, pack=pack_infos, ws=st.ws[1])
        _query_counts(cnt, 0, nc1, num_fine, march_cap, kept_cap)
        depth = torch.empty(march_cap, dtype=torch.float32, device=dev)
        ridx32 = torch.empty(march_cap, dtype=torch.int32, device=dev)
        with L.KERNEL_TIMER.time("march", R):
            if rec_t is not None:
                _call(lib.nsb_march_compact, "march_compact", cnt, CNT_SLOTS["hit"], None, P(rec_t, "f32"), ctypes.c_uint32(max_steps), P(info2, "i32"),
                      P(ridx_hit, "i64"), L.c_i64(R), P(depth), P(ridx32), L.stream_ptr())
            else:
                _call(lib.nsb_ray_marching_listed, "ray_marching", cnt, CNT_SLOTS["hit"], None, *margs, P(info2), None, P(depth), None, P(ridx32), None, None,
                      P(ridx_hit, "i64"), L.c_i64(R), P(bits), L.stream_ptr())
        ridx = ridx32.long()
        from . import neus as GN
        fine_stages = None
        if GN.use_persistent_upsample(R):
            fine_all, _ovf = NF.upsample_rays(st.meta, st.grid16, st.dec, ridx_hit, pack_infos, depth, o_c, d_c, [upsample_inv_s * f for f in factors], num_fine,
                                              max_level=st.ml, max_steps=max_steps, use_estimate_alpha=use_est, collect=st.collect, count=(cnt, CNT_SLOTS["hit"]))
            factors_loop = []
        else:
            factors_loop = factors
        sdf = torch.empty(march_cap if factors_loop else 1, dtype=torch.float32, device=dev)
        if factors_loop:
            fine_stages = []
            order_f = _block_order(rays_inds, ridx_hit, R, cnt, CNT_SLOTS["hit"]) if coherent and n_stage > 1 else None
            _sdf_launch(st.meta, st.grid16, st.dec, o_c, d_c, depth, sdf, ridx=ridx, ml=st.ml, collect=st.collect, cnt=cnt, slot=CNT_SLOTS["marched"])
        for i, factor in enumerate(factors_loop):
            cdf = torch.empty(march_cap, dtype=torch.float32, device=dev)
            _call(lib.nsb_neus_upsample_cdf, "neus_upsample_cdf", cnt, CNT_SLOTS["hit"], None, P(sdf, "f32"), P(depth, "f32"), P(pack_infos, "i64"), L.c_i64(R),
                  L.c_f32(upsample_inv_s * factor), ctypes.c_int(1 if use_est else 0), L.c_f32(1e-4), L.c_f32(0.0), P(cdf), L.stream_ptr())
            nf = num_fine[i]
            fine = torch.empty(R, nf, dtype=torch.float32, device=dev)
            u = NF._U_CACHE.get((nf, dev))
            if u is None:
                u = NF._U_CACHE[(nf, dev)] = torch.linspace(0., 1., nf + 2, device=dev, dtype=torch.float32)[1:-1].contiguous()
            _call(lib.nsb_packed_invert_cdf_shared_u, "packed_invert_cdf_shared_u", cnt, CNT_SLOTS["hit"], None, P(depth, "f32"), P(cdf, "f32"), P(u, "f32"),
                  P(pack_infos, "i64"), L.c_i64(R), L.c_i32(nf), P(fine), L.stream_ptr())
            fine_stages.append(fine)
            if i < n_stage - 1:
                sdf_fine = torch.empty(R * nf, dtype=torch.float32, device=dev)
                if coherent:
                    _sdf_launch(st.meta, st.grid16, st.dec, o_c, d_c, fine.view(-1), sdf_fine, packs=(get_pack_infos_from_batch(R, nf, device=dev), ridx_hit, order_f),
                                ml=st.ml, collect=st.collect, cnt=cnt, slot=CNT_SLOTS["hit"])
                else:
                    _sdf_launch(st.meta, st.grid16, st.dec, o_c, d_c, fine.view(-1), sdf_fine, ridx=ridx_hit.unsqueeze(-1).expand(R, nf).reshape(-1).contiguous(),
                                ml=st.ml, collect=st.collect, cnt=cnt, slot=CNT_SLOTS["fine0"] + i)
                dep_m = torch.empty(march_cap, dtype=torch.float32, device=dev)
                sdf_m = torch.empty(march_cap, dtype=torch.float32, device=dev)
                pim = torch.empty_like(pack_infos)
                _call(lib.nsb_merge_sorted_vals, "merge_sorted_vals", cnt, CNT_SLOTS["hit"], None, P(depth, "f32"), P(sdf, "f32"), P(pack_infos, "i64"),
                      P(fine, "f32"), P(sdf_fine, "f32"), L.c_i64(R), L.c_i32(nf), P(dep_m), P(sdf_m), P(pim), L.stream_ptr())
                depth, sdf, pack_infos = dep_m, sdf_m, pim
        if fine_stages is not None:
            fine_all = (torch.cat(fine_stages, dim=-1) if n_stage > 1 else fine_stages[0]).contiguous()
        d1 = torch.empty(S_cap, dtype=torch.float32, device=dev)
        mid = torch.empty(S_cap, dtype=torch.float32, device=dev)
        ridx_all = torch.empty(S_cap, dtype=torch.int64, device=dev)
        pinfo = torch.empty(R, 2, dtype=torch.int64, device=dev)
        rl = (ctypes.c_int32 * n_stage)(*num_fine)
        _call(lib.nsb_assemble_boundary, "assemble_boundary", cnt, CNT_SLOTS["n_rays"], CNT_SLOTS["hit"], P(coarse, "f32"), L.c_i64(R), L.c_i32(nc1),
              P(ridx_hit, "i64"), L.c_i64(R), P(fine_all, "f32"), L.c_i32(nf_tot), rl, L.c_i32(n_stage), P(d1), P(mid), P(ridx_all), P(pinfo), L.stream_ptr())
    s, b = model.implicit_surface, model.radiance_net.blocks.layers
    dl = s.decoder.layers
    sdf_b = _StaticSDF.apply(st, ridx_all, d1, (pinfo, None, order_b) if coherent else None, CNT_SLOTS["n_rays"] if coherent else CNT_SLOTS["boundary"],
                             s.encoding.flattened_params, dl[0].weight, dl[0].bias, dl[1].weight, dl[1].bias)
    inv_s = model.forward_inv_s()
    if not isinstance(inv_s, torch.Tensor):
        inv_s = torch.tensor(float(inv_s), device=dev)
    alpha, sel, steps = _StaticAlpha.apply(sdf_b, inv_s, pinfo, cnt, 1e-4, 0.0)
    with torch.no_grad():
        first = torch.empty(R, dtype=torch.int32, device=dev)
        nidx = torch.empty(R, dtype=torch.int64, device=dev)
        pinfo_kept = torch.empty(R, 2, dtype=torch.int64, device=dev)
        rays_inds_hit = torch.empty(R, dtype=torch.int64, device=dev)
        _scan(steps, cnt, CNT_SLOTS["kept_raw"], first=first, index=nidx, pack=pinfo_kept, src=rays_inds, nz_src=rays_inds_hit, ws=st.ws[2])
        _query_counts(cnt, 1, nc1, num_fine, march_cap, kept_cap)
        pidx, ridx_k = torch.empty(kept_cap, dtype=torch.int64, device=dev), torch.empty(kept_cap, dtype=torch.int64, device=dev)
        t_k, alpha_c = torch.empty(kept_cap, dtype=torch.float32, device=dev), torch.empty(kept_cap, dtype=torch.float32, device=dev)
        _call(lib.nsb_compact_samples, "compact_samples", cnt, CNT_SLOTS["rays_if_kept_fits"], None, P(sel.view(torch.uint8), "u8"), P(pinfo, "i64"), P(first, "i32"),
              P(steps, "i32"), L.c_i64(R), P(ridx_all, "i64"), P(mid, "f32"), P(alpha.detach(), "f32"), P(pidx), P(ridx_k), P(t_k), P(alpha_c), L.stream_ptr())
    alpha_k = _StaticGather.apply(alpha, pidx, alpha_c, cnt) if alpha.requires_grad else alpha_c
    params = (s.encoding.flattened_params, dl[0].weight, dl[0].bias, dl[1].weight, dl[1].bias, b[0].weight, b[0].bias, b[1].weight, b[1].bias,
              b[2].weight, b[2].bias)
    keep_acts = torch.is_grad_enabled() and any(p.requires_grad for p in params)
    _sdf_k, nab, rgb, x = _StaticColor.apply(st, ridx_k, t_k, view_dirs, ha_c, keep_acts, *params)
    if not nablas_has_grad:
        nab = nab.detach()
    nab_i = nab if with_normal else None
    if nab_i is not None and not training:
        nab_i = F.normalize(nab_i.clamp(-1, 1), dim=-1)
    vw, m, d, c, nn_ = _StaticComposite.apply(alpha_k, t_k, rgb if with_rgb else None, nab_i, pinfo_kept, rays_inds_hit, R, cnt,
                                              bool(depth_use_normalized_vw), 1e-4, 0.0)
    rendered = dict(mask_volume=m, depth_volume=d)
    if with_rgb:
        rendered["rgb_volume"] = c
    if with_normal:
        rendered["normals_volume"] = nn_
    buffers = dict(opacity_alpha=alpha_k, t=t_k, rgb=rgb, nablas=nab, net_x=x, vw=vw, pack_infos_hit=pinfo_kept, rays_inds_hit=rays_inds_hit, ridx=ridx_k,
                   pack_infos_boundary=pinfo, march_pack_infos=pack_infos)
    return rendered, cnt, buffers


def sliced_volume_buffer(buffers, cnt):
    c = cnt.tolist()
    K, Pu = c[CNT_SLOTS["kept"]], c[CNT_SLOTS["kept_rays"]]
    if c[CNT_SLOTS["overflow"]]:
        raise RuntimeError(f"static step: arena overflow (flags {c[CNT_SLOTS['overflow']]}: 1 = marched samples, 2 = kept samples)")
    if K == 0:
        return dict(type="empty", rays_inds_hit=[])
    vb = dict(type="packed", rays_inds_hit=buffers["rays_inds_hit"][:Pu], pack_infos_hit=buffers["pack_infos_hit"][:Pu])
    for k in ("opacity_alpha", "t", "rgb", "nablas", "net_x", "vw"):
        vb[k] = buffers[k][:K]
    return vb


class StaticFrame:

    def __init__(self, model, n_rays, loss_fn=None, *, near=None, far=None, with_rgb=True, with_normal=True, slack=1.5, march_cap=None, kept_cap=None,
                 coherent=None, use_graph=True, zero_grads=False, h_appear_dim=None, pre_hook=None):
        self.model, self.n_rays, self.loss_fn = model, int(n_rays), loss_fn
        self.near, self.far, self.with_rgb, self.with_normal, self.slack = near, far, with_rgb, with_normal, float(slack)
        self.march_cap, self.kept_cap, self.coherent = march_cap, kept_cap, coherent
        self.use_graph, self.zero_grads, self.pre_hook = use_graph, zero_grads, pre_hook
        dev = model.device
        self.device = dev
        self.rays_o = torch.zeros(self.n_rays, 3, device=dev)
        self.rays_d = torch.zeros(self.n_rays, 3, device=dev)
        na = h_appear_dim if h_appear_dim is not None else (model.radiance_net.blocks.layers[0].in_features - 54 if model.use_h_appear else 0)
        self.h_appear = torch.zeros(self.n_rays, na, device=dev) if na > 0 else None
        self.cnt = torch.zeros(32, dtype=torch.int64, device=dev)
        self.graph, self.loss, self.rendered, self.buffers, self._occ_captured = None, None, None, None, None
        self.captures = 0

    @torch.no_grad()
    def _probe(self):
        from ..renderer import SingleVolumeRenderer
        r = SingleVolumeRenderer(dict(near=self.near, far=self.far, with_rgb=self.with_rgb, with_normal=self.with_normal))
        r.train(self.model.training)
        out = r.ray_query(self.model, self.rays_o, self.rays_d, self.h_appear, return_buffer=True, return_details=True)
        det, vb = out.get("details", {}), out["volume_buffer"]
        qp = dict(self.model.ray_query_cfg.get("query_param", {}) or {})
        nf = qp.get("num_fine", 8)
        nf = [nf] * len(qp.get("upsample_inv_s_factors", (1, 4, 16))) if isinstance(nf, int) else list(nf)
        nf = [n // 2 * 2 + 1 for n in nf]
        M = int(det["march.num_per_ray"].sum()) if "march.num_per_ray" in det else 0
        n_hit = int(det["march.num_per_ray"].shape[0]) if "march.num_per_ray" in det else 0
        K = int(vb["t"].shape[0]) if vb.get("type") == "packed" else 0
        return M + n_hit * sum(nf[:-1]), K, bool(out["ray_tested"].get("rays_coherent", False))

    def _size(self, grow=1.0):
        need_m, need_k, coh = self._probe()
        if self.coherent is None:
            self.coherent = coh
        floor = 4096 + 8 * min(self.n_rays, 65536)
        m = int(max(need_m * self.slack, floor) * grow)
        k = int(max(need_k * self.slack, floor) * grow)
        self.march_cap = max(self.march_cap or 0, m)
        self.kept_cap = max(self.kept_cap or 0, k)

    def _run(self):
        if self.pre_hook is not None:
            self.pre_hook()
        if self.zero_grads:
            for p in self.model.parameters():
                if p.grad is not None:
                    p.grad.zero_()
        cv = getattr(self.model, "ctrl_var", None)
        if cv is not None and hasattr(cv, "mix_weight"):
            if getattr(cv, "_w_dev", None) is None:
                cv._w_dev = torch.zeros((), device=self.device)
            cv._use_w_dev = True
        try:
            rendered, _, buffers = render_static(self.model, self.rays_o, self.rays_d, self.h_appear, near=self.near, far=self.far, march_cap=self.march_cap,
                                                 kept_cap=self.kept_cap, coherent=bool(self.coherent), with_rgb=self.with_rgb, with_normal=self.with_normal, cnt=self.cnt)
        finally:
            if cv is not None:
                cv._use_w_dev = False
        loss = None
        if self.loss_fn is not None:
            loss = self.loss_fn(rendered)
            if loss.requires_grad:
                loss.backward()
            loss = loss.detach()
        return rendered, buffers, loss

    def capture(self):
        if self.march_cap is None or self.kept_cap is None or self.coherent is None:
            self._size()
        if not self.use_graph:
            self.graph = None
            return self
        if not bool(self.rays_d.any()):
            raise RuntimeError("StaticFrame.capture: the input buffers hold no rays yet; call step(rays_o, rays_d, ...) or fill frame.rays_o / frame.rays_d first")
        was = L.KERNEL_TIMER.enabled
        L.KERNEL_TIMER.enabled = False
        import gc
        gc.collect()
        try:
            side = torch.cuda.Stream(device=self.device)
            side.wait_stream(torch.cuda.current_stream())
            with torch.cuda.stream(side):
                for _ in range(2):
                    self._run()
            torch.cuda.current_stream().wait_stream(side)
            torch.cuda.synchronize()
            g = torch.cuda.CUDAGraph()
            self._occ_captured = self.model.accel.occ.occ_grid
            with torch.cuda.graph(g, stream=side):
                self.rendered, self.buffers, self.loss = self._run()
            self.graph = g
            self.captures += 1
        finally:
            L.KERNEL_TIMER.enabled = was
        return self

    def step(self, rays_o, rays_d, rays_h_appear=None):
        self.rays_o.copy_(rays_o, non_blocking=True)
        self.rays_d.copy_(rays_d, non_blocking=True)
        if self.h_appear is not None and rays_h_appear is not None:
            self.h_appear.copy_(rays_h_appear, non_blocking=True)
        cv = getattr(self.model, "ctrl_var", None)
        if cv is not None and hasattr(cv, "mix_weight"):
            if getattr(cv, "_w_dev", None) is None:
                cv._w_dev = torch.zeros((), device=self.device)
            cv._w_dev.fill_(cv.mix_weight())
        if self.graph is None and (self.use_graph or self.march_cap is None):
            self.capture()
        if self.graph is not None:
            occ = self.model.accel.occ.occ_grid
            if self._occ_captured is not None and occ.data_ptr() != self._occ_captured.data_ptr():
                self._occ_captured.copy_(occ)
            self.graph.replay()
        else:
            self.rendered, self.buffers, self.loss = self._run()
        return self.loss

    def counts(self):
        c = self.cnt.tolist()
        return {k: c[v] for k, v in CNT_SLOTS.items()}

    def check(self, retry=True):
        if int(self.cnt[CNT_SLOTS["overflow"]]) == 0:
            return True
        self.march_cap = self.kept_cap = None
        self._size(grow=1.25)
        self.graph = None
        if self.use_graph:
            self.capture()
        if retry:
            if self.graph is not None:
                self.graph.replay()
            else:
                self.rendered, self.buffers, self.loss = self._run()
        return False

    def volume_buffer(self):
        return sliced_volume_buffer(self.buffers, self.cnt)
```

profiles/torch_profile_step.py:

```python
import os
import sys

import torch
from torch.profiler import ProfilerActivity, profile

sys.path.insert(0, os.path.dirname(os.path.dirname(os.path.abspath(__file__))))
import bench
from neuralsim_b200.renderer import SingleVolumeRenderer

dev = torch.device("cuda:0")
model = bench.build_model(dev).train()
r = SingleVolumeRenderer(dict(near=0.01)).train()
flat, params = bench.flat_grad_views(model)
o, d = bench.pinhole_rays(bench.H, bench.W, bench.orbit(0, 8))
o, d = o.to(dev), d.to(dev)
CH = int(os.environ.get("CHUNK", 480000))
ha = torch.zeros(CH, 4, device=dev)


def step():
    flat.zero_()
    for s in range(0, o.shape[0], CH):
        e = min(s + CH, o.shape[0])
        out = r.render(model, o[s:e], d[s:e], rays_h_appear=ha[:e - s])["rendered"]
        loss = bench.loss_of(out) * ((e - s) / o.shape[0])
        if loss.requires_grad:
            loss.backward()


for _ in range(2):
    step()
torch.cuda.synchronize()
with profile(activities=[ProfilerActivity.CPU, ProfilerActivity.CUDA]) as prof:
    step()
    torch.cuda.synchronize()
print(prof.key_averages().table(sort_by="self_cuda_time_total", row_limit=45, max_name_column_width=70))
```

Before: 27.91.

## Restrict boundary SDF backward to kept samples and drop mid/ridx buffers

Replaces the full-boundary alpha backward with a kernel that only visits kept samples and their predecessors, counts nonzero SDF gradients per ray, scans them, and builds a compact index list for the fused SDF backward. Midpoint depths and per-sample ray indices are computed on the fly in compaction instead of being materialised in assemble_boundary, and the boundary SDF/alpha/compaction path is wrapped in a single autograd function. The intent is to cut backward work and memory traffic over boundary samples, at the cost of an extra scan and list-building kernel.

Measured after the change: 28.89, median of 6. 3.5% higher.

```diff
diff --git a/include/neuralsim_b200.h b/include/neuralsim_b200.h
--- a/include/neuralsim_b200.h
+++ b/include/neuralsim_b200.h
@@ -159,6 +159,12 @@
                            float alpha_thre, float *alpha, uint8_t *selector, int32_t *num_steps, void *stream);
 int nsb_neus_alpha_backward(const float *sdf, const int64_t *pack_infos, int64_t n_packs, const float *inv_s_dev, const float *d_alpha,
                             float *d_sdf, float *d_inv_s, void *stream);
+int nsb_neus_alpha_backward_kept(const float *sdf, const int64_t *pack_infos, const int64_t *nidx, const int64_t *pack_infos_kept,
+                                 const int64_t *pidx, int64_t n_packs, const float *inv_s_dev, const float *d_alpha, float *d_sdf,
+                                 int32_t *counts, float *d_inv_s, void *stream);
+int nsb_neus_alpha_backward_kept_list(const int64_t *pack_infos, const int64_t *nidx, const int64_t *pack_infos_kept, const int64_t *pidx,
+                                      const float *d_alpha, const float *d_sdf, const int32_t *offsets, int64_t n_packs, int64_t *list,
+                                      int64_t *ray, void *stream);
 int nsb_composite_forward(const float *alpha, const float *t, const float *rgb, const float *nablas, const int64_t *pack_infos,
                           int64_t n_packs, float early_stop_eps, float alpha_thre, int normalize_depth, const int64_t *ray_index,
                           float *vw, float *mask, float *depth, float *rgb_out, float *nablas_out, void *stream);
@@ -178,8 +184,8 @@
                           int32_t n_fine, const int32_t *run_len_host, int32_t n_runs, float *d1, float *mid, int64_t *ridx_all,
                           int64_t *pack_infos, void *stream);
 int nsb_compact_samples(const uint8_t *selector, const int64_t *pack_infos, const int32_t *first_out, const int32_t *kept, int64_t n_packs,
-                        const int64_t *ridx_all, const float *t, const float *alpha, int64_t *pidx, int64_t *ridx_c, float *t_c,
-                        float *alpha_c, void *stream);
+                        const int64_t *ridx_all, const float *t, const float *d1, const float *alpha, int64_t *pidx, int64_t *ridx_c,
+                        float *t_c, float *alpha_c, void *stream);
 int nsb_scatter_f32(const float *src, const int64_t *idx, int64_t n, float *dst, void *stream);
 int nsb_ray_test_aabb(const float *rays_o, const float *rays_d, int64_t n, const float *center3, const float *radius3, int has_near,
                       float near_clip, int has_far, float far_clip, float *o_n, float *d_n, float *near, float *far, int32_t *flag,
diff --git a/neuralsim_b200/csrc/neus_fused.cu b/neuralsim_b200/csrc/neus_fused.cu
--- a/neuralsim_b200/csrc/neus_fused.cu
+++ b/neuralsim_b200/csrc/neus_fused.cu
@@ -93,6 +93,26 @@
     }
 }
 
+__device__ __forceinline__ float alpha_bwd_at(const float *__restrict__ sdf, int64_t b, int64_t n, int64_t k, float inv_s, float g_own,
+                                              float g_prev, float &acc_invs) {
+    const float s = sdf[b + k];
+    const float c = sigmoidf_(s * inv_s);
+    float gc = 0.f;
+    if (k < n - 1) {
+        const float c1 = sigmoidf_(sdf[b + k + 1] * inv_s);
+        const float den = c + 1e-5f;
+        if ((c - c1) / den >= 0.f) gc += g_own * (c1 + 1e-5f) / (den * den);
+    }
+    if (k > 0) {
+        const float cp = sigmoidf_(sdf[b + k - 1] * inv_s);
+        const float den = cp + 1e-5f;
+        if ((cp - c) / den >= 0.f) gc -= g_prev / den;
+    }
+    const float dc = c * (1.f - c);
+    acc_invs += gc * dc * s;
+    return gc * dc * inv_s;
+}
+
 __global__ void __launch_bounds__(kNB)
 k_neus_alpha_bwd(const float *__restrict__ sdf, const int64_t *__restrict__ pi, int64_t n_packs, const float *__restrict__ inv_s_p,
                  const float *__restrict__ d_alpha, float *__restrict__ d_sdf, float *__restrict__ d_inv_s, const int64_t *__restrict__ n_dev) {
@@ -105,26 +125,89 @@
         for (int64_t k = lane; k < n; k += 32) {
             const float g_own = (k < n - 1) ? d_alpha[b + k] : 0.f, g_prev = (k > 0) ? d_alpha[b + k - 1] : 0.f;
             if (g_own == 0.f && g_prev == 0.f) { d_sdf[b + k] = 0.f; continue; }
-            const float s = sdf[b + k];
-            const float c = sigmoidf_(s * inv_s);
-            float gc = 0.f;
-            if (k < n - 1) {
-                const float c1 = sigmoidf_(sdf[b + k + 1] * inv_s);
-                const float den = c + 1e-5f;
-                if ((c - c1) / den >= 0.f) gc += g_own * (c1 + 1e-5f) / (den * den);
-            }
-            if (k > 0) {
-                const float cp = sigmoidf_(sdf[b + k - 1] * inv_s);
-                const float den = cp + 1e-5f;
-                if ((cp - c) / den >= 0.f) gc -= g_prev / den;
-            }
-            const float dc = c * (1.f - c);
-            d_sdf[b + k] = gc * dc * inv_s;
-            acc_invs += gc * dc * s;
+            d_sdf[b + k] = alpha_bwd_at(sdf, b, n, k, inv_s, g_own, g_prev, acc_invs);
         }
     }
     acc_invs = warp_sum(acc_invs);
     if (lane == 0 && acc_invs != 0.f) atomicAdd(d_inv_s, acc_invs);
+}
+
+struct KeptCand {
+    int64_t k[2];
+    float g_own[2], g_prev[2];
+    bool live[2];
+};
+
+__device__ __forceinline__ KeptCand kept_candidates(const int64_t *__restrict__ pidx, const float *__restrict__ d_alpha, int64_t o0, int64_t m,
+                                                    int64_t q, int64_t b, int64_t n) {
+    KeptCand c;
+    c.live[0] = c.live[1] = false;
+    if (q >= m) return c;
+    const int64_t k = pidx[o0 + q] - b;
+    const float g = d_alpha[o0 + q];
+    const bool prev_kept = q > 0 && pidx[o0 + q - 1] - b == k - 1;
+    const bool next_kept = q + 1 < m && pidx[o0 + q + 1] - b == k + 1;
+    c.k[0] = k;
+    c.g_own[0] = (k < n - 1) ? g : 0.f;
+    c.g_prev[0] = prev_kept ? d_alpha[o0 + q - 1] : 0.f;
+    c.live[0] = !(c.g_own[0] == 0.f && c.g_prev[0] == 0.f);
+    c.k[1] = k + 1;
+    c.g_own[1] = 0.f;
+    c.g_prev[1] = g;
+    c.live[1] = k < n - 1 && !next_kept && g != 0.f;
+    return c;
+}
+
+__global__ void __launch_bounds__(kNB)
+k_neus_alpha_bwd_kept(const float *__restrict__ sdf, const int64_t *__restrict__ pi, const int64_t *__restrict__ nidx,
+                      const int64_t *__restrict__ pinfo_kept, const int64_t *__restrict__ pidx, int64_t n_cap, const float *__restrict__ inv_s_p,
+                      const float *__restrict__ d_alpha, float *__restrict__ d_sdf, int32_t *__restrict__ counts, float *__restrict__ d_inv_s,
+                      const int64_t *__restrict__ n_dev) {
+    const int lane = threadIdx.x & 31;
+    const float inv_s = inv_s_p[0];
+    const int64_t live = eff_n(n_cap, n_dev);
+    for (int64_t j = live + (int64_t)blockIdx.x * blockDim.x + threadIdx.x; j < n_cap; j += (int64_t)gridDim.x * blockDim.x) counts[j] = 0;
+    float acc_invs = 0.f;
+    for (int64_t j = gwarp(); j < live; j += nwarps()) {
+        const int64_t p = nidx[j], b = pi[2 * p], n = pi[2 * p + 1], o0 = pinfo_kept[2 * j], m = pinfo_kept[2 * j + 1];
+        int nz = 0;
+        for (int64_t q = lane; q - lane < m; q += 32) {
+            const KeptCand c = kept_candidates(pidx, d_alpha, o0, m, q, b, n);
+#pragma unroll
+            for (int e = 0; e < 2; ++e) {
+                if (!c.live[e]) continue;
+                const float d = alpha_bwd_at(sdf, b, n, c.k[e], inv_s, c.g_own[e], c.g_prev[e], acc_invs);
+                d_sdf[b + c.k[e]] = d;
+                nz += d != 0.f;
+            }
+        }
+        nz = __reduce_add_sync(0xffffffffu, nz);
+        if (lane == 0) counts[j] = nz;
+    }
+    acc_invs = warp_sum(acc_invs);
+    if (lane == 0 && acc_invs != 0.f) atomicAdd(d_inv_s, acc_invs);
+}
+
+__global__ void __launch_bounds__(kNB)
+k_neus_alpha_bwd_kept_list(const int64_t *__restrict__ pi, const int64_t *__restrict__ nidx, const int64_t *__restrict__ pinfo_kept,
+                           const int64_t *__restrict__ pidx, const float *__restrict__ d_alpha, const float *__restrict__ d_sdf,
+                           const int32_t *__restrict__ offs, int64_t n_packs, int64_t *__restrict__ list, int64_t *__restrict__ ray,
+                           const int64_t *__restrict__ n_dev) {
+    const int lane = threadIdx.x & 31;
+    n_packs = eff_n(n_packs, n_dev);
+    for (int64_t j = gwarp(); j < n_packs; j += nwarps()) {
+        const int64_t p = nidx[j], b = pi[2 * p], n = pi[2 * p + 1], o0 = pinfo_kept[2 * j], m = pinfo_kept[2 * j + 1];
+        int64_t out = offs[j];
+        for (int64_t q = lane; q - lane < m; q += 32) {
+            const KeptCand c = kept_candidates(pidx, d_alpha, o0, m, q, b, n);
+            const bool f0 = c.live[0] && d_sdf[b + c.k[0]] != 0.f, f1 = c.live[1] && d_sdf[b + c.k[1]] != 0.f;
+            const uint32_t m0 = __ballot_sync(0xffffffffu, f0), m1 = __ballot_sync(0xffffffffu, f1), lt = (1u << lane) - 1u;
+            const int64_t o = out + __popc(m0 & lt) + __popc(m1 & lt);
+            if (f0) { list[o] = b + c.k[0]; ray[b + c.k[0]] = p; }
+            if (f1) { list[o + f0] = b + c.k[1]; ray[b + c.k[1]] = p; }
+            out += __popc(m0) + __popc(m1);
+        }
+    }
 }
 
 __global__ void __launch_bounds__(kNB)
@@ -269,6 +352,30 @@
     return check_launch("nsb_neus_alpha_backward");
 }
 
+extern "C" int nsb_neus_alpha_backward_kept(const float *sdf, const int64_t *pack_infos, const int64_t *nidx, const int64_t *pack_infos_kept,
+                                            const int64_t *pidx, int64_t n_packs, const float *inv_s_dev, const float *d_alpha, float *d_sdf,
+                                            int32_t *counts, float *d_inv_s, void *stream) {
+    const DevCounts dn = take_counts();
+    if (n_packs == 0) return 0;
+    NSB_REQUIRE(sdf && pack_infos && nidx && pack_infos_kept && pidx && inv_s_dev && d_alpha && d_sdf && counts && d_inv_s,
+                "nsb_neus_alpha_backward_kept: NULL argument");
+    k_neus_alpha_bwd_kept<<<pack_grid(n_packs), kNB, 0, STREAM>>>(sdf, pack_infos, nidx, pack_infos_kept, pidx, n_packs, inv_s_dev, d_alpha, d_sdf,
+                                                                  counts, d_inv_s, dn.a);
+    return check_launch("nsb_neus_alpha_backward_kept");
+}
+
+extern "C" int nsb_neus_alpha_backward_kept_list(const int64_t *pack_infos, const int64_t *nidx, const int64_t *pack_infos_kept, const int64_t *pidx,
+                                                 const float *d_alpha, const float *d_sdf, const int32_t *offsets, int64_t n_packs, int64_t *list,
+                                                 int64_t *ray, void *stream) {
+    const DevCounts dn = take_counts();
+    if (n_packs == 0) return 0;
+    NSB_REQUIRE(pack_infos && nidx && pack_infos_kept && pidx && d_alpha && d_sdf && offsets && list && ray,
+                "nsb_neus_alpha_backward_kept_list: NULL argument");
+    k_neus_alpha_bwd_kept_list<<<pack_grid(n_packs), kNB, 0, STREAM>>>(pack_infos, nidx, pack_infos_kept, pidx, d_alpha, d_sdf, offsets, n_packs, list,
+                                                                       ray, dn.a);
+    return check_launch("nsb_neus_alpha_backward_kept_list");
+}
+
 extern "C" int nsb_composite_forward(const float *alpha, const float *t, const float *rgb, const float *nablas, const int64_t *pack_infos,
                                      int64_t n_packs, float early_stop_eps, float alpha_thre, int normalize_depth, const int64_t *ray_index,
                                      float *vw, float *mask, float *depth, float *rgb_out, float *nablas_out, void *stream) {
diff --git a/neuralsim_b200/csrc/neus_glue.cu b/neuralsim_b200/csrc/neus_glue.cu
--- a/neuralsim_b200/csrc/neus_glue.cu
+++ b/neuralsim_b200/csrc/neus_glue.cu
@@ -164,6 +164,11 @@
 constexpr int kAsmWarps = 8, kAsmMaxRuns = 8, kAsmChunk = 8;
 struct AsmRuns { int n, len[kAsmMaxRuns]; };
 
+__device__ __forceinline__ float interval_mid(float v, float next, bool last) {
+    const float diff = last ? 0.f : __fsub_rn(next, v);
+    return __fadd_rn(v, __fmul_rn(diff, 0.5f));
+}
+
 __device__ __forceinline__ int count_less(const float *a, int n, float v, bool or_equal) {
     int lo = 0, cnt = n;
     while (cnt > 0) {
@@ -207,10 +212,9 @@
             if (!hit) {
                 for (int k = lane; k < nc; k += 32) {
                     const float v = coarse[r * nc + k];
-                    const float diff = (k < nc - 1) ? __fsub_rn(coarse[r * nc + k + 1], v) : 0.f;
                     d1[first + k] = v;
-                    mid[first + k] = __fadd_rn(v, __fmul_rn(diff, 0.5f));
-                    ridx_all[first + k] = r;
+                    if (mid) mid[first + k] = interval_mid(v, k < nc - 1 ? coarse[r * nc + k + 1] : 0.f, k == nc - 1);
+                    if (ridx_all) ridx_all[first + k] = r;
                 }
                 continue;
             }
@@ -233,10 +237,9 @@
             __syncwarp();
             for (int k = lane; k < n; k += 32) {
                 const float v = srt[k];
-                const float diff = (k < n - 1) ? __fsub_rn(srt[k + 1], v) : 0.f;
                 d1[first + k] = v;
-                mid[first + k] = __fadd_rn(v, __fmul_rn(diff, 0.5f));
-                ridx_all[first + k] = r;
+                if (mid) mid[first + k] = interval_mid(v, k < n - 1 ? srt[k + 1] : 0.f, k == n - 1);
+                if (ridx_all) ridx_all[first + k] = r;
             }
         }
     }
@@ -245,7 +248,7 @@
 __global__ void __launch_bounds__(256)
 k_compact_samples(const uint8_t *__restrict__ selector, const int64_t *__restrict__ pi, const int32_t *__restrict__ first_out,
                   const int32_t *__restrict__ kept, int64_t n_packs, const int64_t *__restrict__ ridx_all, const float *__restrict__ t,
-                  const float *__restrict__ alpha, int64_t *__restrict__ pidx, int64_t *__restrict__ ridx_c, float *__restrict__ t_c,
+                  const float *__restrict__ d1, const float *__restrict__ alpha, int64_t *__restrict__ pidx, int64_t *__restrict__ ridx_c, float *__restrict__ t_c,
                   float *__restrict__ alpha_c, const int64_t *__restrict__ n_dev) {
     const int lane = threadIdx.x & 31;
     n_packs = eff_n(n_packs, n_dev);
@@ -262,8 +265,8 @@
             if (sel) {
                 const int64_t o = out + __popc(m & ((1u << lane) - 1u));
                 pidx[o] = b + k;
-                ridx_c[o] = ridx_all[b + k];
-                t_c[o] = t[b + k];
+                ridx_c[o] = ridx_all ? ridx_all[b + k] : p;
+                t_c[o] = t ? t[b + k] : interval_mid(d1[b + k], k < n - 1 ? d1[b + k + 1] : 0.f, k == n - 1);
                 alpha_c[o] = alpha[b + k];
             }
             const int c = __popc(m);
@@ -523,7 +526,7 @@
                                      int64_t *pack_infos, void *stream) {
     const DevCounts dn = take_counts();
     if (n_rays == 0) return 0;
-    NSB_REQUIRE(coarse && d1 && mid && ridx_all && pack_infos, "nsb_assemble_boundary: NULL argument");
+    NSB_REQUIRE(coarse && d1 && pack_infos, "nsb_assemble_boundary: NULL argument");
     NSB_REQUIRE(n_hit == 0 || (ridx_hit && fine), "nsb_assemble_boundary: hit rays need ridx_hit and fine");
     NSB_REQUIRE(n_coarse > 0 && n_fine >= 0 && n_coarse + n_fine <= 1024, "nsb_assemble_boundary: n_coarse + n_fine must be <= 1024");
     const size_t smem = (size_t)kAsmWarps * 2 * (n_coarse + n_fine) * sizeof(float);
@@ -542,14 +545,14 @@
 }
 
 extern "C" int nsb_compact_samples(const uint8_t *selector, const int64_t *pack_infos, const int32_t *first_out, const int32_t *kept, int64_t n_packs,
-                                   const int64_t *ridx_all, const float *t, const float *alpha, int64_t *pidx, int64_t *ridx_c, float *t_c,
-                                   float *alpha_c, void *stream) {
+                                   const int64_t *ridx_all, const float *t, const float *d1, const float *alpha, int64_t *pidx, int64_t *ridx_c,
+                                   float *t_c, float *alpha_c, void *stream) {
     const DevCounts dn = take_counts();
     if (n_packs == 0) return 0;
-    NSB_REQUIRE(selector && pack_infos && first_out && kept && ridx_all && t && alpha && pidx && ridx_c && t_c && alpha_c,
+    NSB_REQUIRE(selector && pack_infos && first_out && kept && (t || d1) && alpha && pidx && ridx_c && t_c && alpha_c,
                 "nsb_compact_samples: NULL argument");
-    k_compact_samples<<<wave_grid(n_packs * 32, 256, 8), 256, 0, STREAM>>>(selector, pack_infos, first_out, kept, n_packs, ridx_all, t, alpha, pidx, ridx_c,
-                                                                          t_c, alpha_c, dn.a);
+    k_compact_samples<<<wave_grid(n_packs * 32, 256, 8), 256, 0, STREAM>>>(selector, pack_infos, first_out, kept, n_packs, ridx_all, t, d1, alpha, pidx,
+                                                                          ridx_c, t_c, alpha_c, dn.a);
     return check_launch("nsb_compact_samples");
 }
 
diff --git a/neuralsim_b200/graphics/neus_fused.py b/neuralsim_b200/graphics/neus_fused.py
--- a/neuralsim_b200/graphics/neus_fused.py
+++ b/neuralsim_b200/graphics/neus_fused.py
@@ -201,7 +201,7 @@
         pidx, ridx_c = torch.empty(K, dtype=torch.int64, device=dev), torch.empty(K, dtype=torch.int64, device=dev)
         t_c, alpha_c = torch.empty(K, dtype=torch.float32, device=dev), torch.empty(K, dtype=torch.float32, device=dev)
         L.check(L.lib().nsb_compact_samples(L.ptr(sel.view(torch.uint8), "u8"), L.ptr(pack_infos, "i64"), L.ptr(sc["first"], "i32"), L.ptr(steps, "i32"),
-                                            L.c_i64(pack_infos.shape[0]), L.ptr(ridx_all, "i64"), L.ptr(t_mid, "f32"), L.ptr(alpha.detach(), "f32"),
+                                            L.c_i64(pack_infos.shape[0]), L.ptr(ridx_all, "i64"), L.ptr(t_mid, "f32"), None, L.ptr(alpha.detach(), "f32"),
                                             L.ptr(pidx), L.ptr(ridx_c), L.ptr(t_c), L.ptr(alpha_c), L.stream_ptr()), "compact_samples")
     alpha_k = _GatherUnique.apply(alpha, pidx, alpha_c) if alpha.requires_grad else alpha_c
     return dict(alpha=alpha_k, ridx=ridx_c, t=t_c, pack_infos=sc["pack"], nidx=sc["index"], rays_inds_hit=sc["src"], pidx=pidx)
diff --git a/neuralsim_b200/graphics/neus_static.py b/neuralsim_b200/graphics/neus_static.py
--- a/neuralsim_b200/graphics/neus_static.py
+++ b/neuralsim_b200/graphics/neus_static.py
@@ -76,87 +76,69 @@
     return order
 
 
-class _StaticSDF(torch.autograd.Function):
+class _StaticBoundary(torch.autograd.Function):
 
     @staticmethod
-    def forward(ctx, st, ridx, t, packs, count_slot, grid, W1, b1, W2, b2):
-        sdf = torch.empty(t.numel(), dtype=torch.float32, device=t.device)
-        _sdf_launch(st.meta, st.grid16, st.dec, st.rays_o, st.rays_d, t, sdf, ridx=ridx if packs is None else None, packs=packs, ml=st.ml,
-                    collect=st.collect, cnt=st.cnt, slot=count_slot, timer="fused_sdf_fwd")
-        ctx.st, ctx.ridx, ctx.t = st, ridx, t
-        ctx.shapes = (grid.shape, W1.shape, b1.shape, W2.shape, b2.shape)
-        return sdf
+    def forward(ctx, st, d1, pinfo, ridx_all, order_b, rays_inds, kept_cap, qc, inv_s, grid, W1, b1, W2, b2):
+        R, dev, cnt, P, lib = pinfo.shape[0], d1.device, st.cnt, L.ptr, L.lib()
+        sdf = torch.empty(d1.numel(), dtype=torch.float32, device=dev)
+        _sdf_launch(st.meta, st.grid16, st.dec, st.rays_o, st.rays_d, d1, sdf, ridx=ridx_all, packs=(pinfo, None, order_b) if ridx_all is None else None,
+                    ml=st.ml, collect=st.collect, cnt=cnt, slot=CNT_SLOTS["n_rays"] if ridx_all is None else CNT_SLOTS["boundary"], timer="fused_sdf_fwd")
+        inv_c = inv_s.detach().contiguous().float().reshape(1)
+        alpha = torch.empty_like(sdf)
+        sel = torch.empty(sdf.shape[0], dtype=torch.bool, device=dev)
+        steps = torch.empty(R, dtype=torch.int32, device=dev)
+        _call(lib.nsb_neus_alpha_forward, "neus_alpha_forward", cnt, CNT_SLOTS["n_rays"], None, P(sdf, "f32"), P(pinfo, "i64"), L.c_i64(R),
+              P(inv_c, "f32"), L.c_f32(1e-4), L.c_f32(0.0), P(alpha), P(sel), P(steps), L.stream_ptr())
+        first = torch.empty(R, dtype=torch.int32, device=dev)
+        nidx = torch.empty(R, dtype=torch.int64, device=dev)
+        pinfo_kept = torch.empty(R, 2, dtype=torch.int64, device=dev)
+        rays_inds_hit = torch.empty(R, dtype=torch.int64, device=dev)
+        _scan(steps, cnt, CNT_SLOTS["kept_raw"], first=first, index=nidx, pack=pinfo_kept, src=rays_inds, nz_src=rays_inds_hit, ws=st.ws[2])
+        _query_counts(cnt, 1, *qc)
+        pidx, ridx_k = torch.empty(kept_cap, dtype=torch.int64, device=dev), torch.empty(kept_cap, dtype=torch.int64, device=dev)
+        t_k, alpha_k = torch.empty(kept_cap, dtype=torch.float32, device=dev), torch.empty(kept_cap, dtype=torch.float32, device=dev)
+        _call(lib.nsb_compact_samples, "compact_samples", cnt, CNT_SLOTS["rays_if_kept_fits"], None, P(sel.view(torch.uint8), "u8"), P(pinfo, "i64"),
+              P(first, "i32"), P(steps, "i32"), L.c_i64(R), None, None, P(d1, "f32"), P(alpha, "f32"), P(pidx), P(ridx_k), P(t_k), P(alpha_k), L.stream_ptr())
+        ctx.st, ctx.saved = st, (d1, sdf, inv_c, pinfo, nidx, pinfo_kept, pidx)
+        ctx.shapes = (inv_s.shape, grid.shape, W1.shape, b1.shape, W2.shape, b2.shape)
+        ctx.mark_non_differentiable(t_k, ridx_k, pinfo_kept, rays_inds_hit)
+        return alpha_k, t_k, ridx_k, pinfo_kept, rays_inds_hit
 
     @staticmethod
     @torch.autograd.function.once_differentiable
-    def backward(ctx, d_sdf):
-        st, dev = ctx.st, d_sdf.device
-        gs, w1s, b1s, w2s, b2s = ctx.shapes
+    def backward(ctx, g_alpha, _gt, _gr, _gp, _gi):
+        st, (d1, sdf, inv_c, pinfo, nidx, pinfo_kept, pidx) = ctx.st, ctx.saved
+        dev, R, S, K = sdf.device, pinfo.shape[0], sdf.numel(), pidx.numel()
+        inv_shape, gs, w1s, b1s, w2s, b2s = ctx.shapes
         d_grid = torch.zeros(gs, dtype=torch.float32, device=dev)
         ks = [int(torch.Size(x).numel()) for x in (w1s, b1s, w2s, b2s)]
-        small = torch.zeros(sum(ks), dtype=torch.float32, device=dev)
-        d_W1, d_b1 = small[:ks[0]].view(w1s), small[ks[0]:ks[0] + ks[1]].view(b1s)
-        d_W2, d_b2 = small[ks[0] + ks[1]:ks[0] + ks[1] + ks[2]].view(w2s), small[ks[0] + ks[1] + ks[2]:].view(b2s)
-        d_sdf = d_sdf.contiguous().float()
-        n = d_sdf.numel()
-        P, cnt = L.ptr, st.cnt
-        flag = torch.empty(n, dtype=torch.int32, device=dev)
-        _call(L.lib().nsb_flag_nonzero, "flag_nonzero", cnt, CNT_SLOTS["boundary"], None, P(d_sdf, "f32"), L.c_i64(n), P(flag), L.stream_ptr())
-        keep = torch.empty(n, dtype=torch.int64, device=dev)
-        _scan(flag, cnt, CNT_SLOTS["nonzero"], index=keep, ws=st.ws[3])
-        with L.KERNEL_TIMER.time("fused_sdf_bwd", n):
-            _call(L.lib().nsb_fused_sdf_bwd_indexed, "fused_sdf_bwd", cnt, CNT_SLOTS["nonzero"], None,
-                  st.meta.c_ref, P(st.grid16, "f16"), ctypes.byref(st.dec), None, P(st.rays_o, "f32"), P(st.rays_d, "f32"), P(ctx.ridx, "i64"),
-                  P(ctx.t, "f32"), P(d_sdf, "f32"), P(keep, "i64"), L.c_i64(n), L.c_i32(st.ml), P(d_grid), P(d_W1), P(d_b1), P(d_W2), P(d_b2),
-                  L.stream_ptr())
-        return None, None, None, None, None, d_grid, d_W1, d_b1, d_W2, d_b2
-
-
-class _StaticAlpha(torch.autograd.Function):
-
-    @staticmethod
-    def forward(ctx, sdf, inv_s, pack_infos, cnt, early_stop_eps, alpha_thre):
-        sdf_c, inv_c = sdf.detach().contiguous().float(), inv_s.detach().contiguous().float().reshape(1)
-        Pn, dev = pack_infos.shape[0], sdf_c.device
-        alpha = torch.empty_like(sdf_c)
-        sel = torch.empty(sdf_c.shape[0], dtype=torch.bool, device=dev)
-        steps = torch.empty(Pn, dtype=torch.int32, device=dev)
-        P = L.ptr
-        _call(L.lib().nsb_neus_alpha_forward, "neus_alpha_forward", cnt, CNT_SLOTS["n_rays"], None, P(sdf_c, "f32"), P(pack_infos, "i64"), L.c_i64(Pn),
-              P(inv_c, "f32"), L.c_f32(early_stop_eps), L.c_f32(alpha_thre), P(alpha), P(sel), P(steps), L.stream_ptr())
-        ctx.save_for_backward(sdf_c, inv_c, pack_infos)
-        ctx.cnt, ctx.inv_shape = cnt, inv_s.shape
-        ctx.mark_non_differentiable(sel, steps)
-        return alpha, sel, steps
-
-    @staticmethod
-    def backward(ctx, g_alpha, _gs, _gn):
-        sdf_c, inv_c, pack_infos = ctx.saved_tensors
-        g = g_alpha.contiguous().float()
-        d_sdf = torch.empty_like(sdf_c)
-        d_inv = torch.zeros(1, device=sdf_c.device, dtype=torch.float32)
-        P = L.ptr
-        _call(L.lib().nsb_neus_alpha_backward, "neus_alpha_backward", ctx.cnt, CNT_SLOTS["n_rays"], None, P(sdf_c, "f32"), P(pack_infos, "i64"),
-              L.c_i64(pack_infos.shape[0]), P(inv_c, "f32"), P(g, "f32"), P(d_sdf), P(d_inv), L.stream_ptr())
-        return (d_sdf if ctx.needs_input_grad[0] else None, d_inv.reshape(ctx.inv_shape) if ctx.needs_input_grad[1] else None, None, None, None, None)
-
-
-class _StaticGather(torch.autograd.Function):
-
-    @staticmethod
-    def forward(ctx, src, pidx, gathered, cnt):
-        ctx.save_for_backward(pidx)
-        ctx.n, ctx.cnt = src.shape[0], cnt
-        return gathered
-
-    @staticmethod
-    def backward(ctx, g):
-        pidx, = ctx.saved_tensors
-        g = g.contiguous().float()
-        d = torch.zeros(ctx.n, dtype=torch.float32, device=g.device)
-        P = L.ptr
-        _call(L.lib().nsb_scatter_f32, "scatter_f32", ctx.cnt, CNT_SLOTS["kept"], None, P(g, "f32"), P(pidx, "i64"), L.c_i64(pidx.shape[0]), P(d), L.stream_ptr())
-        return d, None, None, None
+        small = torch.zeros(1 + sum(ks), dtype=torch.float32, device=dev)
+        d_inv, o = small[:1], 1
+        d_W1, d_b1 = small[o:o + ks[0]].view(w1s), small[o + ks[0]:o + ks[0] + ks[1]].view(b1s)
+        o += ks[0] + ks[1]
+        d_W2, d_b2 = small[o:o + ks[2]].view(w2s), small[o + ks[2]:].view(b2s)
+        P, cnt, lib = L.ptr, st.cnt, L.lib()
+        if g_alpha is not None:
+            g = g_alpha.contiguous().float()
+            d_sdf = torch.empty(S, dtype=torch.float32, device=dev)
+            ray = torch.empty(S, dtype=torch.int64, device=dev)
+            counts = torch.empty(R, dtype=torch.int32, device=dev)
+            a = (P(pinfo, "i64"), P(nidx, "i64"), P(pinfo_kept, "i64"), P(pidx, "i64"))
+            _call(lib.nsb_neus_alpha_backward_kept, "neus_alpha_backward_kept", cnt, CNT_SLOTS["kept_rays"], None, P(sdf, "f32"), *a, L.c_i64(R),
+                  P(inv_c, "f32"), P(g, "f32"), P(d_sdf), P(counts), P(d_inv), L.stream_ptr())
+            offs = torch.empty(R, dtype=torch.int32, device=dev)
+            _scan(counts, cnt, CNT_SLOTS["nonzero"], first=offs, ws=st.ws[3])
+            n_list = min(S, 2 * K)
+            keep = torch.empty(n_list, dtype=torch.int64, device=dev)
+            _call(lib.nsb_neus_alpha_backward_kept_list, "neus_alpha_backward_kept_list", cnt, CNT_SLOTS["kept_rays"], None, *a, P(g, "f32"), P(d_sdf, "f32"),
+                  P(offs, "i32"), L.c_i64(R), P(keep), P(ray), L.stream_ptr())
+            with L.KERNEL_TIMER.time("fused_sdf_bwd", n_list):
+                _call(lib.nsb_fused_sdf_bwd_indexed, "fused_sdf_bwd", cnt, CNT_SLOTS["nonzero"], None,
+                      st.meta.c_ref, P(st.grid16, "f16"), ctypes.byref(st.dec), None, P(st.rays_o, "f32"), P(st.rays_d, "f32"), P(ray, "i64"),
+                      P(d1, "f32"), P(d_sdf, "f32"), P(keep, "i64"), L.c_i64(n_list), L.c_i32(st.ml), P(d_grid), P(d_W1), P(d_b1), P(d_W2), P(d_b2),
+                      L.stream_ptr())
+        return (None,) * 8 + (d_inv.reshape(inv_shape), d_grid, d_W1, d_b1, d_W2, d_b2)
 
 
 class _StaticColor(torch.autograd.Function):
@@ -429,32 +411,20 @@
         if fine_stages is not None:
             fine_all = (torch.cat(fine_stages, dim=-1) if n_stage > 1 else fine_stages[0]).contiguous()
         d1 = torch.empty(S_cap, dtype=torch.float32, device=dev)
-        mid = torch.empty(S_cap, dtype=torch.float32, device=dev)
-        ridx_all = torch.empty(S_cap, dtype=torch.int64, device=dev)
+        ridx_all = None if coherent else torch.empty(S_cap, dtype=torch.int64, device=dev)
         pinfo = torch.empty(R, 2, dtype=torch.int64, device=dev)
         rl = (ctypes.c_int32 * n_stage)(*num_fine)
         _call(lib.nsb_assemble_boundary, "assemble_boundary", cnt, CNT_SLOTS["n_rays"], CNT_SLOTS["hit"], P(coarse, "f32"), L.c_i64(R), L.c_i32(nc1),
-              P(ridx_hit, "i64"), L.c_i64(R), P(fine_all, "f32"), L.c_i32(nf_tot), rl, L.c_i32(n_stage), P(d1), P(mid), P(ridx_all), P(pinfo), L.stream_ptr())
+              P(ridx_hit, "i64"), L.c_i64(R), P(fine_all, "f32"), L.c_i32(nf_tot), rl, L.c_i32(n_stage), P(d1), None, P(ridx_all, "i64", allow_none=True), P(pinfo),
+              L.stream_ptr())
     s, b = model.implicit_surface, model.radiance_net.blocks.layers
     dl = s.decoder.layers
-    sdf_b = _StaticSDF.apply(st, ridx_all, d1, (pinfo, None, order_b) if coherent else None, CNT_SLOTS["n_rays"] if coherent else CNT_SLOTS["boundary"],
-                             s.encoding.flattened_params, dl[0].weight, dl[0].bias, dl[1].weight, dl[1].bias)
     inv_s = model.forward_inv_s()
     if not isinstance(inv_s, torch.Tensor):
         inv_s = torch.tensor(float(inv_s), device=dev)
-    alpha, sel, steps = _StaticAlpha.apply(sdf_b, inv_s, pinfo, cnt, 1e-4, 0.0)
-    with torch.no_grad():
-        first = torch.empty(R, dtype=torch.int32, device=dev)
-        nidx = torch.empty(R, dtype=torch.int64, device=dev)
-        pinfo_kept = torch.empty(R, 2, dtype=torch.int64, device=dev)
-        rays_inds_hit = torch.empty(R, dtype=torch.int64, device=dev)
-        _scan(steps, cnt, CNT_SLOTS["kept_raw"], first=first, index=nidx, pack=pinfo_kept, src=rays_inds, nz_src=rays_inds_hit, ws=st.ws[2])
-        _query_counts(cnt, 1, nc1, num_fine, march_cap, kept_cap)
-        pidx, ridx_k = torch.empty(kept_cap, dtype=torch.int64, device=dev), torch.empty(kept_cap, dtype=torch.int64, device=dev)
-        t_k, alpha_c = torch.empty(kept_cap, dtype=torch.float32, device=dev), torch.empty(kept_cap, dtype=torch.float32, device=dev)
-        _call(lib.nsb_compact_samples, "compact_samples", cnt, CNT_SLOTS["rays_if_kept_fits"], None, P(sel.view(torch.uint8), "u8"), P(pinfo, "i64"), P(first, "i32"),
-              P(steps, "i32"), L.c_i64(R), P(ridx_all, "i64"), P(mid, "f32"), P(alpha.detach(), "f32"), P(pidx), P(ridx_k), P(t_k), P(alpha_c), L.stream_ptr())
-    alpha_k = _StaticGather.apply(alpha, pidx, alpha_c, cnt) if alpha.requires_grad else alpha_c
+    alpha_k, t_k, ridx_k, pinfo_kept, rays_inds_hit = _StaticBoundary.apply(
+        st, d1, pinfo, ridx_all, order_b, rays_inds, kept_cap,
+        (nc1, num_fine, march_cap, kept_cap), inv_s, s.encoding.flattened_params, dl[0].weight, dl[0].bias, dl[1].weight, dl[1].bias)
     params = (s.encoding.flattened_params, dl[0].weight, dl[0].bias, dl[1].weight, dl[1].bias, b[0].weight, b[0].bias, b[1].weight, b[1].bias,
               b[2].weight, b[2].bias)
     keep_acts = torch.is_grad_enabled() and any(p.requires_grad for p in params)
diff --git a/profiles/torch_profile_step.py b/profiles/torch_profile_step.py
--- a/profiles/torch_profile_step.py
+++ b/profiles/torch_profile_step.py
@@ -1,3 +1,5 @@
+import argparse
+import json
 import os
 import sys
 
@@ -5,20 +7,35 @@
 from torch.profiler import ProfilerActivity, profile
 
 sys.path.insert(0, os.path.dirname(os.path.dirname(os.path.abspath(__file__))))
+sys.path.insert(0, os.path.dirname(os.path.abspath(__file__)))
 import bench
+from bwd_kernels import gpu_info
+from neuralsim_b200 import _lib
 from neuralsim_b200.renderer import SingleVolumeRenderer
+
+ap = argparse.ArgumentParser()
+ap.add_argument("--static", action="store_true")
+ap.add_argument("--steps", type=int, default=5)
+args = ap.parse_args()
 
 dev = torch.device("cuda:0")
 model = bench.build_model(dev).train()
 r = SingleVolumeRenderer(dict(near=0.01)).train()
 flat, params = bench.flat_grad_views(model)
-o, d = bench.pinhole_rays(bench.H, bench.W, bench.orbit(0, 8))
+o, d = bench.pinhole_rays(bench.H, bench.W, bench.orbit(0, bench.N_VIEWS if args.static else 8))
 o, d = o.to(dev), d.to(dev)
 CH = int(os.environ.get("CHUNK", 480000))
 ha = torch.zeros(CH, 4, device=dev)
+frame = None
+if args.static:
+    from neuralsim_b200.graphics.neus_static import StaticFrame
+    frame = StaticFrame(model, o.shape[0], loss_fn=bench.loss_of, near=0.01, use_graph=False, pre_hook=flat.zero_)
 
 
 def step():
+    if frame is not None:
+        frame.step(o, d, None)
+        return
     flat.zero_()
     for s in range(0, o.shape[0], CH):
         e = min(s + CH, o.shape[0])
@@ -28,10 +45,32 @@
             loss.backward()
 
 
-for _ in range(2):
+for _ in range(3):
     step()
 torch.cuda.synchronize()
-with profile(activities=[ProfilerActivity.CPU, ProfilerActivity.CUDA]) as prof:
-    step()
+if not args.static:
+    with profile(activities=[ProfilerActivity.CPU, ProfilerActivity.CUDA]) as prof:
+        step()
+        torch.cuda.synchronize()
+    print(prof.key_averages().table(sort_by="self_cuda_time_total", row_limit=45, max_name_column_width=70))
+    sys.exit(0)
+
+l0 = _lib.launch_count()
+step()
+torch.cuda.synchronize()
+launches = _lib.launch_count() - l0
+with profile(activities=[ProfilerActivity.CUDA]) as prof:
+    for _ in range(args.steps):
+        step()
     torch.cuda.synchronize()
-print(prof.key_averages().table(sort_by="self_cuda_time_total", row_limit=45, max_name_column_width=70))
+rows = {}
+for e in prof.key_averages():
+    us = getattr(e, "self_device_time_total", None) or getattr(e, "self_cuda_time_total", 0.0)
+    if us > 0:
+        name = e.key.split("(")[0].replace("void ", "").split("<")[0].strip()
+        rt = rows.setdefault(name, [0.0, 0])
+        rt[0] += us / 1e3 / args.steps
+        rt[1] += e.count / args.steps
+table = sorted(([k, round(v[0], 4), v[1]] for k, v in rows.items()), key=lambda x: -x[1])
+print(json.dumps(dict(ms_per_step_total=round(sum(x[1] for x in table), 3), nsb_launches_per_step=launches, steps=args.steps,
+                      kernels=table, **gpu_info())))
```
